# ZooMEISTER/vickers-hardness-Unet

Measured on AMD Instinct MI355X. Metric: 512x512 images/sec (train fwd+bwd), higher is better.
Workload: dtype bf16

## Files before the change

### vickers-hardness-unet_amd/csrc/conv_halo.hip

```cpp
#include <stdlib.h>
#include <string.h>

#include <string>
#include <type_traits>

#include "vk_common.h"

#ifdef VK_STAMP
#define VK_T(var) { __builtin_amdgcn_sched_barrier(0); const unsigned long long t_ = __builtin_amdgcn_s_memtime(); __builtin_amdgcn_s_waitcnt(0xC07F); __builtin_amdgcn_sched_barrier(0); var = t_; }
#else
#define VK_T(var)
#endif

namespace vk {

struct HaloSrc {
  const void* ptr;
  const float* scale;
  const float* shift;
  int C, up, relu;
  uint32_t bytes;
};

#ifndef VK_EPI_BATCH_READS
#define VK_EPI_BATCH_READS 1
#endif
#ifndef VK_COLP_DEFER_STATS
#define VK_COLP_DEFER_STATS 1
#endif
#ifndef VK_COLQ_ILV
#define VK_COLQ_ILV 1
#endif
#ifndef VK_COLQ_DIAG
#define VK_COLQ_DIAG 0
#endif
#ifndef VK_COLQ_PRE
#define VK_COLQ_PRE 1
#endif
struct HaloParams {
  HaloSrc s0, s1;
  const void* w;
  uint32_t w_bytes;
  void* y0;
  void* y1;
  int ld0, ld1, split;
  double* stats;
  int N, H, W, K, C, flip, accumulate, pool2;
  int Hi, Wi;
  int tiles_x, tiles_y, nchunks;
  unsigned long long* stamps;
  int kyn;
  int ksplit;
  size_t slab_bytes;
  float* slab;
  int dbg;
  const void* bnr_z;
  const float* bnr_scale;
  const float* bnr_shift;
  double* bnr_sums;
  const void* bnr_mask;
};

template <typename T, int TH, int BN, int WGM, int WGN>
struct HaloCfg {
  using Tr = ElemTraits<T>;
  static constexpr int EB = Tr::kBytes;
  static constexpr int VE = Tr::kVec;
  static constexpr int CK = 64 / EB;
  static constexpr int HW_ = 18, HH = TH + 2, HPIX = HH * HW_;
  static constexpr int APS = 96;
  static constexpr int A_BYTES = HPIX * APS;
  static constexpr int B_BYTES = 3 * BN * 64;
  static constexpr int NPV = (HPIX * 4 + 255) / 256;
  static constexpr int NBV = (3 * BN * 4 + 255) / 256;
  static constexpr int BM = TH * 16;
  static constexpr int WR = TH / WGM;
  static constexpr int WCH = BN / WGN;
  static constexpr int TP = WR, TC = WCH / 16;
  static constexpr int ESB = BN * EB + 16;
  static constexpr int EVPR = BN / VE;
  static constexpr int ERPP = 256 / EVPR;
  static constexpr int EPASS = BM / ERPP;
  static constexpr int RED_OFF = BM * ESB;
  static constexpr int MAIN = A_BYTES + 2 * B_BYTES;
  static constexpr int ESLOTS = (BN / VE > 16) ? 4 * 4 / (BN / VE / 16) : 4 * 4;
  static constexpr int EPI = RED_OFF + ESLOTS * BN * 2 * 4;
  static constexpr int SMEM = MAIN > EPI ? MAIN : EPI;
  static_assert(WGM * WGN == 4 && TH % WGM == 0 && BN % (16 * WGN) == 0, "wave layout");
  static_assert(EPASS >= 1, "epilogue mapping");
  static_assert(SMEM <= 160 * 1024, "main-loop / epilogue LDS image exceeds the 160 KiB of a CU");
};

__device__ __forceinline__ int swz(int row) { return ((row >> 2) & 1) << 1; }

__device__ __forceinline__ int halo_group(int tid) {
  const int g = tid >> 2;
  return (g & ~3) | ((g & 1) << 1) | ((g >> 1) & 1);
}


template <typename T, int TH, int BN, int TP, int TC, int NT = 256, bool PRE = false, int OS = 1>
__device__ __forceinline__ void halo_epilogue(char* smem, f32x4_t (&acc)[TC][TP], const HaloParams& p, int n, int y0, int x0, int n0,
                                              int wrow0, int wch0, int py = 0, int px = 0, double* defer = nullptr) {
  using Tr = ElemTraits<T>;
  constexpr int EB = Tr::kBytes, VE = Tr::kVec;
  constexpr int BM = TH * 16;
  constexpr int ESB = BN * EB + 16;
  constexpr int EVPR = BN / VE, ERPP = NT / EVPR, EPASS = BM / ERPP, NW = NT / 64;
  constexpr int RED_OFF = BM * ESB;
  static_assert(BM % ERPP == 0 && EVPR <= 64, "epilogue mapping");
  const int tid = threadIdx.x, lane = tid & 63, wave = tid >> 6;
  const int li = lane & 15, kg = lane >> 4;

  const int e_row = tid / EVPR;
  const int e_vec = (EVPR == 16 && EB == 2) ? (((tid & 15) + ((e_row & 1) ? 15 : 0)) & 15) : tid % EVPR;
  const int col0 = n0 + e_vec * VE;
  const bool col_ok = col0 < p.K;
  char* yb = (char*)p.y0;
  int ld = p.ld0, colx = col0;
  bool first_part = true;
  if (p.split > 0 && col0 >= p.split) { yb = (char*)p.y1; ld = p.ld1; colx = col0 - p.split; first_part = false; }
  float s1[VE], s2[VE];
#pragma unroll
  for (int j = 0; j < VE; ++j) { s1[j] = 0.f; s2[j] = 0.f; }
  const bool bnr = p.bnr_z != nullptr && first_part && col_ok;
  const bool ext_mask = p.bnr_mask != nullptr;
  float bsc[VE], bsh[VE];
  if (bnr && !ext_mask) {
#pragma unroll
    for (int j = 0; j < VE; ++j) { bsc[j] = p.bnr_scale[colx + j]; bsh[j] = p.bnr_shift[colx + j]; }
  }
  auto finish = [&](float (&f)[VE], size_t elem_off, const u32x4_t* pre_old, const u32x4_t* pre_z, const u32x4_t* pre_m = nullptr) {
    u32x4_t* gp = reinterpret_cast<u32x4_t*>(yb + elem_off * EB);
    if (p.accumulate) {
      float o[VE];
      Vec16<T>::unpack(pre_old ? *pre_old : *gp, o);
#pragma unroll
      for (int j = 0; j < VE; ++j) f[j] += o[j];
    }
    u32x4_t v = Vec16<T>::pack(f);
    Vec16<T>::unpack(v, f);
    if (bnr) {
      float zf[VE];
// ... 73 lines not shown
        for (int q = 0; q < 4; ++q) {
          const int row = (2 * py + (q >> 1)) * 16 + 2 * px + (q & 1);
          float t[VE];
          Vec16<T>::unpack(*reinterpret_cast<const u32x4_t*>(smem + row * ESB + e_vec * 16), t);
#pragma unroll
          for (int j = 0; j < VE; ++j) f[j] += t[j];
        }
        finish(f, (((size_t)n * Hh + y) * Wh + x) * ld + colx, nullptr, nullptr);
      }
    }
  } else if (p.accumulate || p.bnr_z != nullptr) {
#pragma unroll
    for (int ps = 0; ps < EPASS; ++ps) {
      const int row = e_row + ps * ERPP;
      const int y = OS * (y0 + (row >> 4)) + py, x = OS * (x0 + (row & 15)) + px;
      if (y < p.H && x < p.W && col_ok) {
        const u32x4_t raw = *reinterpret_cast<const u32x4_t*>(smem + row * ESB + e_vec * 16);
        const size_t eoff = (((size_t)n * p.H + y) * p.W + x) * ld + colx;
        float f[VE];
        Vec16<T>::unpack(raw, f);
        if (PRE) finish(f, eoff, &oldv[ps], &zv[ps], PRE_M ? &mv[ps] : nullptr);
        else finish(f, eoff, nullptr, nullptr);
      }
    }
  } else {
    constexpr int RB = VK_EPI_BATCH_READS ? (EPASS < 8 ? EPASS : 8) : 1;
    u32x4_t raws[RB];
#pragma unroll
    for (int ps = 0; ps < EPASS; ++ps) {
      if (ps % RB == 0) {
#pragma unroll
        for (int q = 0; q < RB; ++q)
          if (ps + q < EPASS) raws[q] = *reinterpret_cast<const u32x4_t*>(smem + (e_row + (ps + q) * ERPP) * ESB + e_vec * 16);
      }
      const int row = e_row + ps * ERPP;
      const int y = OS * (y0 + (row >> 4)) + py, x = OS * (x0 + (row & 15)) + px;
      if (y < p.H && x < p.W && col_ok) {
        const u32x4_t raw = raws[ps % RB];
        const size_t eoff = (((size_t)n * p.H + y) * p.W + x) * ld + colx;
        if (p.stats) {
          float f[VE];
          Vec16<T>::unpack(raw, f);
#pragma unroll
          for (int j = 0; j < VE; ++j) { s1[j] += f[j]; s2[j] += f[j] * f[j]; }
        }
        *reinterpret_cast<u32x4_t*>(yb + eoff * EB) = raw;
      }
    }
  }
  if (p.stats || p.bnr_sums) {
    if (p.bnr_sums && !bnr) {
#pragma unroll
      for (int j = 0; j < VE; ++j) { s1[j] = 0.f; s2[j] = 0.f; }
    }
#pragma unroll
    for (int j = 0; j < VE; ++j) {
      if (EVPR <= 1) { s1[j] += dpp_f<0xB1>(s1[j]); s2[j] += dpp_f<0xB1>(s2[j]); }
      if (EVPR <= 2) { s1[j] += dpp_f<0x4E>(s1[j]); s2[j] += dpp_f<0x4E>(s2[j]); }
      if (EVPR <= 4) { s1[j] += dpp_f<0x124>(s1[j]); s2[j] += dpp_f<0x124>(s2[j]); }
      if (EVPR <= 8) { s1[j] += dpp_f<0x128>(s1[j]); s2[j] += dpp_f<0x128>(s2[j]); }
    }
    float* red = reinterpret_cast<float*>(smem + RED_OFF);
    constexpr int RPS = EVPR > 16 ? EVPR / 16 : 1, NSLOT = NW * 4 / RPS;
    static_assert(EVPR <= 32, "partial-sum slots");
    if (EVPR > 16 || li < EVPR) {
      const int slot = (wave * 4 + kg) / RPS;
#pragma unroll
      for (int j = 0; j < VE; ++j) {
        red[(slot * BN + e_vec * VE + j) * 2 + 0] = s1[j];
        red[(slot * BN + e_vec * VE + j) * 2 + 1] = s2[j];
      }
    }
    __syncthreads();
    if (tid < BN && n0 + tid < p.K) {
      float a = 0.f, b = 0.f;
#pragma unroll
      for (int w = 0; w < NSLOT; ++w) { a += red[(w * BN + tid) * 2]; b += red[(w * BN + tid) * 2 + 1]; }
      if (defer) {
        defer[0] += (double)a;
        defer[1] += (double)b;
      } else if (p.bnr_sums) {
        const int kc = p.ld0;
        if (n0 + tid < kc) {
          double* sp = p.bnr_sums + (size_t)(blockIdx.x % VK_STATS_REPLICAS) * 2 * kc;
          atomicAdd(sp + n0 + tid, (double)a);
          atomicAdd(sp + kc + n0 + tid, (double)b);
        }
      } else {
        double* sp = p.stats + (size_t)(blockIdx.x % VK_STATS_REPLICAS) * 2 * p.K;
        atomicAdd(sp + n0 + tid, (double)a);
        atomicAdd(sp + p.K + n0 + tid, (double)b);
      }
    }
  }
}

template <int BN>
__device__ __forceinline__ void stats_flush(const HaloParams& p, int n0, double (&d)[2]) {
  const int tid = threadIdx.x;
  if (tid < BN && n0 + tid < p.K) {
    if (p.bnr_sums) {
      const int kc = p.ld0;
      if (n0 + tid < kc) {
        double* sp = p.bnr_sums + (size_t)(blockIdx.x % VK_STATS_REPLICAS) * 2 * kc;
        atomicAdd(sp + n0 + tid, d[0]);
        atomicAdd(sp + kc + n0 + tid, d[1]);
      }
    } else if (p.stats) {
      double* sp = p.stats + (size_t)(blockIdx.x % VK_STATS_REPLICAS) * 2 * p.K;
      atomicAdd(sp + n0 + tid, d[0]);
      atomicAdd(sp + p.K + n0 + tid, d[1]);
    }
  }
  d[0] = 0.0;
  d[1] = 0.0;
}

template <typename T, int TH, int BN, int WGM, int WGN>
__global__ __launch_bounds__(256, 2) void conv3x3_halo_kernel(const HaloParams p) {
  using Cfg = HaloCfg<T, TH, BN, WGM, WGN>;
  constexpr int EB = Cfg::EB, VE = Cfg::VE, CK = Cfg::CK, HPIX = Cfg::HPIX, NPV = Cfg::NPV, NBV = Cfg::NBV;
  constexpr int TP = Cfg::TP, TC = Cfg::TC, APS = Cfg::APS;

  extern __shared__ __attribute__((aligned(16))) char smem[];
  char* const Abuf = smem;
  char* const Bbuf = smem + Cfg::A_BYTES;
  const int tid = threadIdx.x, lane = tid & 63, wave = tid >> 6;

  int bt = blockIdx.x;
  if ((gridDim.x & 7) == 0) bt = (bt & 7) * (int)(gridDim.x >> 3) + (bt >> 3);
  const int tx = bt % p.tiles_x;
  bt /= p.tiles_x;
  const int ty = bt % p.tiles_y;
  const int n = bt / p.tiles_y;
  const int y0 = ty * TH, x0 = tx * 16;
  const int n0 = blockIdx.y * BN;

  const __amdgpu_buffer_rsrc_t rs0 = make_rsrc(p.s0.ptr, p.s0.bytes);
  const __amdgpu_buffer_rsrc_t rs1 = make_rsrc(p.s1.ptr ? p.s1.ptr : p.s0.ptr, p.s1.ptr ? p.s1.bytes : 0u);
  const __amdgpu_buffer_rsrc_t rsw = make_rsrc(p.w, p.w_bytes);

  const int hv = tid & 3;
  const int hgrp = halo_group(tid);
  int h_full[NPV], h_half[NPV];
  const int Hh = p.H >> 1, Wh = p.W >> 1;
#pragma unroll
  for (int i = 0; i < NPV; ++i) {
    const int hp = hgrp + i * 64;
    const int hy = hp / 18, hx = hp - hy * 18;
    const int y = y0 - 1 + hy, x = x0 - 1 + hx;
    const bool ok = hp < HPIX && (unsigned)y < (unsigned)p.H && (unsigned)x < (unsigned)p.W;
    h_full[i] = ok ? (n * p.H + y) * p.W + x : -1;
    h_half[i] = ok ? (n * Hh + (y >> 1)) * Wh + (x >> 1) : -1;
  }
  int b_toff[NBV];
  int b_s[NBV];
#pragma unroll
  for (int i = 0; i < NBV; ++i) {
    const int idx = tid + i * 256;
    b_s[i] = idx / (BN * 4);
    b_toff[i] = idx < 3 * BN * 4 ? (idx - b_s[i] * (BN * 4)) * 16 : -1;
  }
  const uint32_t slab_bytes = (uint32_t)p.K * 64u;

  u32x4_t areg[NPV], breg0[NBV], breg1[NBV];
  float sc[VE], sh[VE];
  bool aff = false, relu = false;

  auto load_halo = [&](int cc) {
    const int c = cc * CK;
    const bool first = c < p.s0.C;
    const HaloSrc& sd = first ? p.s0 : p.s1;
    const int cl = (first ? c : c - p.s0.C) + hv * VE;
    aff = sd.scale != nullptr;
    relu = sd.relu != 0;
    if (aff) {
#pragma unroll
      for (int j = 0; j < VE; j += 4) {
        const f32x4_t s4 = *reinterpret_cast<const f32x4_t*>(sd.scale + cl + j);
        const f32x4_t h4 = *reinterpret_cast<const f32x4_t*>(sd.shift + cl + j);
#pragma unroll
        for (int e = 0; e < 4; ++e) { sc[j + e] = s4[e]; sh[j + e] = h4[e]; }
      }
    }
    const bool up = sd.up != 0;
#pragma unroll
    for (int i = 0; i < NPV; ++i) {
      const int pix = up ? h_half[i] : h_full[i];
      const uint32_t off = (uint32_t)(pix * sd.C + cl) * (uint32_t)EB;
      if (first) areg[i] = buf_load16(rs0, pix >= 0 ? off : kOOB);
      else areg[i] = buf_load16(rs1, pix >= 0 ? off : kOOB);
    }
// ... 1265 lines not shown

template <typename T>
__global__ __launch_bounds__(256, 3) void stem7x7_kernel(const HaloParams p) {
  using Cfg = ColCfg<T, 16, 64, 4, 1, false>;
  static_assert(sizeof(T) == 2, "16-bit types: a pixel of the NHWC4 input is 8 bytes");
  constexpr int NV = (StemTile::ROWS * StemTile::VPR + 255) / 256;
  extern __shared__ __attribute__((aligned(16))) char smem[];
  const int tid = threadIdx.x, lane = tid & 63;
  const int wave = __builtin_amdgcn_readfirstlane(tid >> 6);
  int bt = blockIdx.x;
  if ((gridDim.x & 7) == 0) bt = (bt & 7) * (int)(gridDim.x >> 3) + (bt >> 3);
  const int tx = bt % p.tiles_x;
  bt /= p.tiles_x;
  const int ty = bt % p.tiles_y;
  const int n = bt / p.tiles_y;
  const int y0 = ty * 16, x0 = tx * 16;
  const __amdgpu_buffer_rsrc_t rs0 = make_rsrc(p.s0.ptr, p.s0.bytes);
  const __amdgpu_buffer_rsrc_t rsw = make_rsrc(p.w, p.w_bytes);

  u32x4_t areg[NV];
#pragma unroll
  for (int i = 0; i < NV; ++i) {
    const int v = tid + i * 256;
    const int ry = v / StemTile::VPR, vc = v - ry * StemTile::VPR;
    const int y = 2 * y0 - 3 + ry, x = 2 * x0 - 4 + 2 * vc;
    const bool ok = v < StemTile::ROWS * StemTile::VPR && (unsigned)y < (unsigned)p.Hi && (unsigned)x < (unsigned)p.Wi;
    areg[i] = buf_load16(rs0, ok ? (uint32_t)((n * p.Hi + y) * p.Wi + x) * 8u : kOOB);
  }
  const int li = lane & 15, kg = lane >> 4;
  typedef __attribute__((address_space(3))) void lds_void;
  char* const Wl = smem + StemTile::W_OFF;
#pragma unroll
  for (int i = 0; i < 7; ++i) {
    const int pc = wave * 7 + i, r = pc >> 2, a = pc & 3;
    const uint32_t voff = (uint32_t)((((a * 16 + li) * 7 + r) * 32 + kg * 8) * 2);
    __builtin_amdgcn_raw_ptr_buffer_load_lds(rsw, (lds_void*)(Wl + pc * 1024), 16, voff, 0, 0, 0);
  }
#pragma unroll
  for (int i = 0; i < NV; ++i) {
    const int v = tid + i * 256;
    if (v >= StemTile::ROWS * StemTile::VPR) continue;
    const int ry = v / StemTile::VPR, vc = v - ry * StemTile::VPR;
    char* row = smem + ry * StemTile::PITCH;
    if (vc > 0) *reinterpret_cast<u32x2_t*>(row + (2 * vc - 1) * 8) = u32x2_t{areg[i][0], areg[i][1]};
    *reinterpret_cast<u32x2_t*>(row + (2 * vc) * 8) = u32x2_t{areg[i][2], areg[i][3]};
  }
  __syncthreads();

  const int wrow0 = wave * 4;
  f32x4_t acc[4][4];
#pragma unroll
  for (int a = 0; a < 4; ++a)
#pragma unroll
    for (int b = 0; b < 4; ++b) acc[a][b] = f32x4_t{0.f, 0.f, 0.f, 0.f};
  const char* const xl = smem + (2 * wrow0) * StemTile::PITCH + 16 * (li + kg);
  const char* const wl = Wl + lane * 16;
#pragma unroll
  for (int r = 0; r < 7; ++r) {
    u32x4_t X[4], Wc[4];
#pragma unroll
    for (int a = 0; a < 4; ++a) Wc[a] = *reinterpret_cast<const u32x4_t*>(wl + (4 * r + a) * 1024);
#pragma unroll
    for (int b = 0; b < 4; ++b) X[b] = *reinterpret_cast<const u32x4_t*>(xl + (2 * b + r) * StemTile::PITCH);
#pragma unroll
    for (int a = 0; a < 4; ++a)
#pragma unroll
      for (int b = 0; b < 4; ++b) acc[a][b] = Mma<T>::run(Wc[a], X[b], acc[a][b]);
  }
  __syncthreads();
  halo_epilogue<T, 16, 64, 4, 4, 256, false>(smem, acc, p, n, y0, x0, 0, wrow0, 0);
}

int stem_tile_launch(vk_dtype dt, int N, int H, int W, const void* x4, const void* wp, void* y, double* stats, hipStream_t st) {
  if (dt == VK_F32 || getenv("VK_NO_STEM_TILE")) return VK_ERR_UNSUPPORTED;
  if ((size_t)N * H * W * 8 >= (1ull << 31)) return VK_ERR_UNSUPPORTED;
  HaloParams p;
  memset((void*)&p, 0, sizeof(p));
  p.s0 = HaloSrc{x4, nullptr, nullptr, 4, 0, 0, (uint32_t)((size_t)N * H * W * 8)};
  p.w = wp;
  p.w_bytes = 64u * 7u * 32u * 2u;
  p.y0 = y;
  p.ld0 = 64;
  p.stats = stats;
  p.N = N; p.H = H / 2; p.W = W / 2; p.K = 64; p.C = 4;
  p.Hi = H; p.Wi = W;
  p.tiles_x = (p.W + 15) / 16;
  p.tiles_y = (p.H + 15) / 16;
  using Cfg = ColCfg<bf16_t, 16, 64, 4, 1, false>;
  constexpr int MAIN = StemTile::W_OFF + StemTile::W_BYTES;
  constexpr int SMEM = MAIN > Cfg::EPI ? MAIN : Cfg::EPI;
  const dim3 grid((unsigned)(N * p.tiles_y * p.tiles_x));
  vkh::ProfScope ps("stem_tile_16b", st, 2.0 * (double)N * p.H * p.W * 64.0 * 147.0, ((double)N * H * W * 4.0 + (double)N * p.H * p.W * 64.0) * 2.0);
  if (dt == VK_BF16) hipLaunchKernelGGL(stem7x7_kernel<bf16_t>, grid, dim3(256), SMEM, st, p);
  else hipLaunchKernelGGL(stem7x7_kernel<f16_t>, grid, dim3(256), SMEM, st, p);
  VK_CHECK_HIP(hipGetLastError());
  return VK_OK;
}

template <typename T, int BN>
struct C16Cfg {
  static constexpr int TH = 16, HPIX = 18 * 18;
  static constexpr int APS = 48;
  static constexpr int A_BYTES = HPIX * APS + 64;
  static constexpr int BS = 336;
  static constexpr int B_BYTES = BN * BS;
  static constexpr int TP = 4, TC = BN / 16;
  static constexpr int ESB = BN * 2 + 16;
  static constexpr int EPI = 256 * ESB + 4 * 4 * BN * 2 * 4;
  static constexpr int MAIN = A_BYTES + B_BYTES;
  static constexpr int SMEM = MAIN > EPI ? MAIN : EPI;
};

template <typename T, int BN>
__global__ __launch_bounds__(256) void conv3x3_c16_kernel(const HaloParams p) {
  using Cfg = C16Cfg<T, BN>;
  constexpr int TH = 16, HPIX = Cfg::HPIX, APS = Cfg::APS, BS = Cfg::BS, TP = Cfg::TP, TC = Cfg::TC, VE = 8;
  static_assert(sizeof(T) == 2, "C16 kernel is for 16-bit element types (fp32 uses the generic kernel with 16-channel chunks)");
  extern __shared__ __attribute__((aligned(16))) char smem[];
  char* const Abuf = smem;
  char* const Bbuf = smem + Cfg::A_BYTES;
  const int tid = threadIdx.x, lane = tid & 63, wave = tid >> 6;
  int bt = blockIdx.x;
  if ((gridDim.x & 7) == 0) bt = (bt & 7) * (int)(gridDim.x >> 3) + (bt >> 3);
  const int tx = bt % p.tiles_x;
  bt /= p.tiles_x;
  const int ty = bt % p.tiles_y;
  const int n = bt / p.tiles_y;
  const int y0 = ty * TH, x0 = tx * 16;
  const int n0 = blockIdx.y * BN;
  const __amdgpu_buffer_rsrc_t rs0 = make_rsrc(p.s0.ptr, p.s0.bytes);
  const __amdgpu_buffer_rsrc_t rsw = make_rsrc(p.w, p.w_bytes);

  const bool aff = p.s0.scale != nullptr, relu = p.s0.relu != 0;
  const int hv = (tid >> 3) & 1;
  const int hgrp = (tid & 7) | ((tid >> 4) << 3);
  float sc[VE], sh[VE];
#pragma unroll
  for (int j = 0; j < VE; ++j) {
    sc[j] = aff ? p.s0.scale[hv * VE + j] : 1.f;
    sh[j] = aff ? p.s0.shift[hv * VE + j] : 0.f;
  }
  constexpr int NPV = (HPIX * 2 + 255) / 256;
  u32x4_t areg[NPV];
  bool aok[NPV];
#pragma unroll
  for (int i = 0; i < NPV; ++i) {
    const int hp = hgrp + i * 128;
    const int hy = hp / 18, hx = hp - hy * 18;
    const int y = y0 - 1 + hy, x = x0 - 1 + hx;
    aok[i] = hp < HPIX && (unsigned)y < (unsigned)p.H && (unsigned)x < (unsigned)p.W;
    const uint32_t off = (uint32_t)(((n * p.H + y) * p.W + x) * 16 + hv * VE) * 2u;
    areg[i] = buf_load16(rs0, aok[i] ? off : kOOB);
  }
  constexpr int NBV = (BN * 18 + 255) / 256;
  u32x4_t breg[NBV];
#pragma unroll
  for (int i = 0; i < NBV; ++i) {
    const int idx = tid + i * 256;
    const int row = idx / 18, v = idx - row * 18;
    const int tap = p.flip ? 8 - (v >> 1) : (v >> 1);
    const bool ok = idx < BN * 18 && n0 + row < p.K;
    breg[i] = buf_load16(rsw, ok ? (uint32_t)(((n0 + row) * 9 + tap) * 16 + (v & 1) * VE) * 2u : kOOB);
  }
  if (tid < 4) *reinterpret_cast<u32x4_t*>(Abuf + HPIX * APS + tid * 16) = u32x4_t{0, 0, 0, 0};
  if (tid < BN) {
    *reinterpret_cast<u32x4_t*>(Bbuf + tid * BS + 288) = u32x4_t{0, 0, 0, 0};
// ... 262 lines not shown
  issue(jb + 1, pre[1]);
  issue(jb + 2, pre[2]);
  if (BNR) z_issue(POOL ? ys + 1 : ys, zq[0]);
  write_row(jb - 1, pre[3]);
  issue(jb + 3, pre[3]);
  write_row(jb, pre[0]);
  auto row = [&](int y, auto ph_c) {
    constexpr int PH = decltype(ph_c)::value;
    if constexpr (!UP) {
      constexpr int S = (PH + 1) & 3;
      write_row(y + 1, pre[S]);
      issue(y + 4, pre[PH & 3]);
    } else if constexpr ((PH & 1) == 1) {
      constexpr int M1 = ((PH + 1) >> 1) & 3;
      const int m1 = (y + 1) >> 1;
      write_row(m1, pre[M1]);
      issue(m1 + 3, pre[(M1 + 3) & 3]);
    }
    constexpr int ZC = POOL ? ((PH >> 1) & 1) : (PH & 1);
    if constexpr (BNR && (!POOL || (PH & 1) == 1)) z_issue(POOL ? y + 2 : y + 1, zq[ZC ^ 1]);
    f32x4_t acc[TC];
#pragma unroll
    for (int a = 0; a < TC; ++a) acc[a] = f32x4_t{0.f, 0.f, 0.f, 0.f};
#pragma unroll
    for (int st = 0; st < NSTEP; ++st) {
      int addr;
      if (CIN == 16) {
        const int vrow = y - 1 + fr_r16[st];
        addr = fr_r16[st] < 0 ? Cfg::ZERO_OFF : (vrow & 3) * ROWB + fr_off16[st];
      } else {
        const int r = st / 3, sxx = st - r * 3;
        const int vrow = y - 1 + r;
        const int jr = UP ? (vrow >> 1) : vrow;
        const int pix = UP ? ((li + sxx + 1) >> 1) : (li + sxx);
        addr = (jr & 3) * ROWB + pix * APS + fr_base32;
      }
      const u32x4_t xf = *reinterpret_cast<const u32x4_t*>(ring + addr);
#pragma unroll
      for (int a = 0; a < TC; ++a) acc[a] = Mma<T>::run(wf[st][a], xf, acc[a]);
    }
#if !(VK_STREAM_DIAG & 16)
    __builtin_amdgcn_sched_barrier(0);
#endif
    const bool y_ok = y < p.H;
#pragma unroll
    for (int a = 0; a < TC; ++a) {
      const int ch = a * 16 + kg * 4;
      float f[4] = {acc[a][0], acc[a][1], acc[a][2], acc[a][3]};
      u32x2_t pk = round_t(f);
      if constexpr (POOL) {
        if constexpr ((PH & 1) == 0) {
#pragma unroll
          for (int e = 0; e < 4; ++e) prev[a][e] = f[e];
        } else {
          float t[4];
#pragma unroll
          for (int e = 0; e < 4; ++e) {
            const float pn = dpp_f<0xB1>(prev[a][e]), cn = dpp_f<0xB1>(f[e]);
            t[e] = ((prev[a][e] + pn) + f[e]) + cn;
          }
          const u32x2_t pk2 = round_t(t);
          finish(a, t, pk2, y_ok ? out_off(a, y) : kOOB, lane_stores && y_ok, zq[ZC][a]);
        }
      } else {
        finish(a, f, pk, y_ok ? out_off(a, y) : kOOB, lane_stores && y_ok, zq[ZC][a]);
      }
    }
  };
  constexpr int UF = UP ? 8 : 4;
  for (int yb = ys; yb < ye; yb += UF) {
    row(yb, std::integral_constant<int, 0>{});
    row(yb + 1, std::integral_constant<int, 1>{});
    row(yb + 2, std::integral_constant<int, 2>{});
    row(yb + 3, std::integral_constant<int, 3>{});
    if constexpr (UP) {
      row(yb + 4, std::integral_constant<int, 4>{});
      row(yb + 5, std::integral_constant<int, 5>{});
      row(yb + 6, std::integral_constant<int, 6>{});
      row(yb + 7, std::integral_constant<int, 7>{});
    }
  }

  if (want_sums) {
    double* const sp = (p.bnr_sums ? p.bnr_sums : p.stats) + (size_t)(strip % VK_STATS_REPLICAS) * 2 * ld;
#pragma unroll
    for (int a = 0; a < TC; ++a)
#pragma unroll
      for (int e = 0; e < 4; ++e) {
        const float u = row16_sum(s1[a][e]), v = row16_sum(s2[a][e]);
        const int ch = a * 16 + kg * 4 + e;
        if (li == 0 && ch < ld) {
          atomicAdd(sp + ch, (double)u);
          atomicAdd(sp + ld + ch, (double)v);
        }
      }
  }
}

struct TailCfg {
  static constexpr int S_STRIDE = 96, A1_STRIDE = 48, A2_PS = 20;
  static constexpr int S_BYTES = 144 * S_STRIDE;
  static constexpr int A1_BYTES = 400 * A1_STRIDE + 64;
  static constexpr int A2_BYTES = 324 * A2_PS * 4;
  static constexpr int SMEM = S_BYTES + A1_BYTES + A2_BYTES;
};

struct TailParams {
  const void* src;
  const float* s0;
  const float* h0;
  const void* w1;
  const float* s1;
  const float* h1;
  const void* w2;
  const float* s2;
  const float* h2;
  const float* hw;
  const float* hb;
  float* logits;
  int N, H, W;
  uint32_t src_bytes;
};

template <typename T>
__global__ __launch_bounds__(256) void dec4_tail_eval_kernel(const TailParams p) {
  using Cfg = TailCfg;
  static_assert(sizeof(T) == 2, "16-bit element types");
  constexpr int VE = 8;
  extern __shared__ __attribute__((aligned(16))) char smem[];
  char* const Sb = smem;
  char* const A1 = smem + Cfg::S_BYTES;
  float* const A2 = reinterpret_cast<float*>(smem + Cfg::S_BYTES + Cfg::A1_BYTES);
  const int tid = threadIdx.x, lane = tid & 63, wave = tid >> 6, li = lane & 15, kg = lane >> 4;
  const int tiles_x = p.W >> 4, tiles_y = p.H >> 4;
  int bt = blockIdx.x;
  const int tx0 = bt % tiles_x;
  bt /= tiles_x;
  const int ty0 = bt % tiles_y;
  const int n = bt / tiles_y;
  const int y0 = ty0 * 16, x0 = tx0 * 16;
  const int Hs = p.H >> 1, Ws = p.W >> 1;
  const int sy0 = (y0 >> 1) - 2, sx0 = (x0 >> 1) - 2;
  const __amdgpu_buffer_rsrc_t rss = make_rsrc(p.src, p.src_bytes);

  u32x4_t wf1[9], wf2[5];
#pragma unroll
  for (int st = 0; st < 9; ++st) {
    const int pos = kg ^ (((li >> 2) & 1) << 1);
    wf1[st] = *reinterpret_cast<const u32x4_t*>((const char*)p.w1 + ((st * 16 + li) * 4 + pos) * 16);
  }
#pragma unroll
  for (int st = 0; st < 5; ++st) {
    const int tap = 2 * st + (kg >> 1);
    wf2[st] = u32x4_t{0, 0, 0, 0};
    if (tap < 9) wf2[st] = *reinterpret_cast<const u32x4_t*>((const char*)p.w2 + ((li * 9 + tap) * 16 + (kg & 1) * VE) * 2);
  }
  float sc1[8], sh1[8], sc2[4], sh2[4];
#pragma unroll
  for (int e = 0; e < 4; ++e) {
    sc1[e] = p.s1[kg * 4 + e]; sh1[e] = p.h1[kg * 4 + e];
    sc1[4 + e] = 0.f; sh1[4 + e] = 0.f;
    sc2[e] = p.s2[kg * 4 + e]; sh2[e] = p.h2[kg * 4 + e];
  }
  if (tid < 4) *reinterpret_cast<u32x4_t*>(A1 + 400 * Cfg::A1_STRIDE + tid * 16) = u32x4_t{0, 0, 0, 0};

  {
    float sc0[VE], sh0[VE];
// ... 402 lines not shown
  static const std::string tag_f = std::string("stream_16b_c") + std::to_string(CIN) + (UP ? "up" : "") + "_k" + std::to_string(TC * 16);
  static const std::string tag_d = tag_f + "_dgrad";
  const std::string& tag = p.flip ? tag_d : tag_f;
  const double in_px = (double)p.N * (p.H >> (UP ? 1 : 0)) * (p.W >> (UP ? 1 : 0));
  const double out_px = (double)p.N * p.H * p.W * (p.pool2 ? 0.25 : 1.0);
  const double bytes = (in_px * CIN + out_px * p.K * (p.bnr_z ? 2.0 : 1.0) + 9.0 * p.K * CIN) * 2.0;
  vkh::ProfScope ps(tag.c_str(), st, 2.0 * (double)p.N * p.H * p.W * p.K * 9.0 * CIN, bytes);
  hipLaunchKernelGGL((conv3x3_stream_kernel<T, CIN, TC, UP, MODE>), grid, dim3(256), Cfg::SMEM, st, q);
  VK_CHECK_HIP(hipGetLastError());
  return VK_OK;
}

template <typename T>
static int stream_try(const HaloParams& p, hipStream_t st) {
  if (getenv("VK_NO_STREAM")) return VK_ERR_UNSUPPORTED;
  if (p.s1.ptr || p.accumulate || p.split || p.ld0 != p.K) return VK_ERR_UNSUPPORTED;
  const bool up = p.s0.up != 0, bnr = p.bnr_z != nullptr, pool = p.pool2 != 0;
  if ((pool || up) && ((p.H | p.W) & 1)) return VK_ERR_UNSUPPORTED;
  const bool fwd = !p.flip && !bnr && !pool;
  if (fwd && p.C == 32 && up && p.K == 16) return launch_stream<T, 32, 1, true, 0>(p, st);
  if (fwd && p.C == 16 && !up && p.K == 16) return launch_stream<T, 16, 1, false, 0>(p, st);
  if (fwd && p.C == 32 && !up && p.K == 32) return launch_stream<T, 32, 2, false, 0>(p, st);
  if (p.flip && !p.s0.scale && bnr && !pool && p.C == 16 && p.K == 16) return launch_stream<T, 16, 1, false, 2>(p, st);
  if (p.flip && !p.s0.scale && bnr && !pool && p.C == 32 && p.K == 32) return launch_stream<T, 32, 2, false, 2>(p, st);
  if (p.flip && !p.s0.scale && bnr && pool && p.C == 16 && p.K == 32) return launch_stream<T, 16, 2, false, 3>(p, st);
  return VK_ERR_UNSUPPORTED;
}

int conv3x3_halo_try(const vk_conv_desc* d, const void* w, int packed, void* y, void* y1, int split_k1, int accumulate, double* stats,
                     int pool2, const vk_bnr* bnr, hipStream_t st, void* workspace, size_t workspace_bytes) {
  const bool s2 = d->stride == 2 && !d->transposed && d->H == 2 * d->Ho && d->W == 2 * d->Wo && d->K >= 128 && !d->src0.up && !d->src1.ptr &&
                  !pool2 && !bnr && !accumulate && !split_k1 && !getenv("VK_NO_S2_TILE");
  const bool s2d = d->stride == 2 && d->transposed && d->Ho == 2 * d->H && d->Wo == 2 * d->W && d->K >= 64 && d->K % 64 == 0 && !d->src0.up &&
                   !d->src1.ptr && !d->src0.scale && !pool2 && !bnr && !split_k1 && !getenv("VK_NO_S2_TILE");
  if (d->R != 3 || d->S != 3 || d->pad != 1) return VK_ERR_UNSUPPORTED;
  if (!s2 && !s2d && (d->stride != 1 || d->H != d->Ho || d->W != d->Wo)) return VK_ERR_UNSUPPORTED;
  const int eb = d->dtype == VK_F32 ? 4 : 2;
  const int ck = 64 / eb;
  const int C = d->src0.C + (d->src1.ptr ? d->src1.C : 0);
  const bool c16 = (eb == 2) && C == 16 && !d->src1.ptr && !d->src0.up && !s2 && !s2d;
  if (c16 ? packed : !packed) return VK_ERR_UNSUPPORTED;
  if (!c16 && (d->src0.C % ck || (d->src1.ptr && d->src1.C % ck))) return VK_ERR_UNSUPPORTED;
  if (d->K % 16) return VK_ERR_UNSUPPORTED;
  if (pool2 && ((d->H | d->W) & 1)) return VK_ERR_UNSUPPORTED;
  if (d->src1.ptr && d->src1.up) return VK_ERR_UNSUPPORTED;
  if ((size_t)d->N * d->H * d->W * C * eb >= (1ull << 31) || (size_t)d->N * d->H * d->W >= (1ull << 31)) return VK_ERR_UNSUPPORTED;
  if (s2d && (size_t)d->N * d->Ho * d->Wo * d->K * eb >= (1ull << 32)) return VK_ERR_UNSUPPORTED;
  HaloParams p;
  auto mk = [&](const vk_src& s) {
    HaloSrc h;
    h.ptr = s.ptr; h.scale = s.scale; h.shift = s.shift; h.C = s.C; h.up = s.up; h.relu = s.relu;
    h.bytes = s.ptr ? (uint32_t)((size_t)d->N * (d->H >> s.up) * (d->W >> s.up) * s.C * eb) : 0u;
    return h;
  };
  p.s0 = mk(d->src0);
  if (d->src1.ptr) p.s1 = mk(d->src1);
  else p.s1 = HaloSrc{nullptr, nullptr, nullptr, 0, 0, 0, 0u};
  p.w = w;
  p.w_bytes = (uint32_t)((size_t)d->K * 9 * C * eb);
  p.y0 = y; p.y1 = y1; p.split = split_k1;
  p.ld0 = split_k1 ? split_k1 : d->K;
  p.ld1 = split_k1 ? d->K - split_k1 : 0;
  p.stats = stats;
  p.N = d->N; p.H = d->Ho; p.W = d->Wo; p.K = d->K; p.C = C;
  p.Hi = d->H; p.Wi = d->W;
  p.flip = d->transposed;
  p.accumulate = accumulate;
  p.pool2 = pool2;
  p.ksplit = 1;
  p.kyn = 0;
  p.slab = (reinterpret_cast<uintptr_t>(workspace) & 15) ? nullptr : (float*)workspace;
  p.slab_bytes = p.slab ? workspace_bytes : 0;
  p.stamps = nullptr;
  p.dbg = getenv("VK_COL_DBG") ? atoi(getenv("VK_COL_DBG")) : 0;
  if (p.dbg & 1) p.w_bytes = 0;
#ifdef VK_STAMP
  { extern unsigned long long* g_vk_stamp_buf; p.stamps = g_vk_stamp_buf; }
#endif
  p.bnr_z = bnr ? bnr->z : nullptr;
  p.bnr_scale = bnr ? bnr->scale : nullptr;
  p.bnr_shift = bnr ? bnr->shift : nullptr;
  p.bnr_sums = bnr ? bnr->sums : nullptr;
  p.bnr_mask = bnr ? bnr->mask : nullptr;
  p.nchunks = c16 ? 1 : C / ck;
  if (p.bnr_mask && (c16 || s2 || s2d || pool2)) return VK_ERR_UNSUPPORTED;
  if (eb == 2 && !s2 && !s2d && !p.bnr_mask && (c16 || C == 32)) {
    const int rc = d->dtype == VK_BF16 ? stream_try<bf16_t>(p, st) : stream_try<f16_t>(p, st);
    if (rc != VK_ERR_UNSUPPORTED) return rc;
  }
  if (c16) {
    if (d->dtype == VK_BF16) return d->K >= 32 ? launch_c16<bf16_t, 32>(p, st) : launch_c16<bf16_t, 16>(p, st);
    return d->K >= 32 ? launch_c16<f16_t, 32>(p, st) : launch_c16<f16_t, 16>(p, st);
  }
  p.tiles_x = p.tiles_y = 0;
  if (s2d) {
    p.flip = 0;
    const long tiles = (long)d->N * ((d->H + 7) / 8) * ((d->W + 15) / 16);
    const bool wide = d->K % 128 == 0 && tiles * (d->K / 128) >= 256;
    switch (d->dtype) {
      case VK_F32: return wide ? launch_s2dg<float, 128>(p, st) : launch_s2dg<float, 64>(p, st);
      case VK_BF16: return wide ? launch_s2dg<bf16_t, 128>(p, st) : launch_s2dg<bf16_t, 64>(p, st);
      case VK_F16: return wide ? launch_s2dg<f16_t, 128>(p, st) : launch_s2dg<f16_t, 64>(p, st);
    }
    return VK_ERR_ARG;
  }
  if (s2) {
    p.slab = nullptr;
    p.slab_bytes = 0;
    switch (d->dtype) {
      case VK_F32: return launch_col<float, 8, 128, 2, 4, false, 1, 0, 2>(p, st);
      case VK_BF16: return launch_col<bf16_t, 8, 128, 2, 4, false, 1, 0, 2>(p, st);
      case VK_F16: return launch_col<f16_t, 8, 128, 2, 4, false, 1, 0, 2>(p, st);
    }
    return VK_ERR_ARG;
  }
  switch (d->dtype) {
    case VK_F32: return halo_select<float>(p, st);
    case VK_BF16: return halo_select<bf16_t>(p, st);
    case VK_F16: return halo_select<f16_t>(p, st);
  }
  return VK_ERR_ARG;
}

}

extern "C" int vk_dec4_tail_eval(vk_dtype dtype, int N, int H, int W, const vk_src* src, const void* w1_pack, const float* scale1,
                                 const float* shift1, const void* w2_plain, const float* scale2, const float* shift2, const float* head_w9x16,
                                 const float* head_bias, float* logits, void* stream) {
  return vk::dec4_tail_eval_impl(dtype, N, H, W, src, w1_pack, scale1, shift1, w2_plain, scale2, shift2, head_w9x16, head_bias, logits,
                                 (hipStream_t)stream);
}
```

### vickers-hardness-unet_amd/csrc/elementwise.hip

```cpp
#include <math.h>

#include "vk_common.h"

namespace vk {

static inline int grid_for(size_t work_items, int block = 256, int max_blocks = 256 * 16) {
  size_t b = (work_items + block - 1) / block;
  if (b > (size_t)max_blocks) b = max_blocks;
  if (b < 1) b = 1;
  return (int)b;
}

template <typename T>
__global__ void k_input_transform(int N, int H, int W, const float* __restrict__ x, T* __restrict__ x4) {
  const size_t HW = (size_t)H * W;
  const float* xn = x + (size_t)blockIdx.y * 3 * HW;
  T* on = x4 + (size_t)blockIdx.y * HW * 4;
  for (size_t hw = blockIdx.x * (size_t)blockDim.x + threadIdx.x; hw < HW; hw += (size_t)gridDim.x * blockDim.x) {
    const float r = xn[hw], g = xn[HW + hw], b = xn[2 * HW + hw];
    if constexpr (sizeof(T) == 4) {
      *reinterpret_cast<f32x4_t*>(on + hw * 4) = f32x4_t{r, g, b, 0.f};
    } else {
      float f[8] = {r, g, b, 0.f, 0.f, 0.f, 0.f, 0.f};
      const u32x4_t pk = Vec16<T>::pack(f);
      *reinterpret_cast<u32x2_t*>(on + hw * 4) = u32x2_t{pk[0], pk[1]};
    }
  }
}

__global__ __launch_bounds__(256) void k_bn_finalize(int C, int train, const double* __restrict__ stats, double count,
                                                     const float* __restrict__ gamma, const float* __restrict__ beta, float* running_mean,
                                                     float* running_var, float eps, float momentum, float* scale, float* shift,
                                                     float* save_mean, float* save_invstd) {
  static_assert(VK_STATS_REPLICAS == 32, "lane mapping assumes 32 replicas");
  const int c = blockIdx.x * 8 + (threadIdx.x >> 5);
  const int r = threadIdx.x & 31;
  double s1 = 0.0, s2 = 0.0;
  if (train && c < C) {
    s1 = stats[(size_t)r * 2 * C + c];
    s2 = stats[(size_t)r * 2 * C + C + c];
  }
  const bool fin = r == 0 && c < C;
  const float ga = fin ? gamma[c] : 0.f, be = fin ? beta[c] : 0.f;
  const float rm0 = fin && running_mean ? running_mean[c] : 0.f, rv0 = fin && running_var ? running_var[c] : 0.f;
#pragma unroll
  for (int o = 16; o > 0; o >>= 1) {
    s1 += __shfl_xor(s1, o, 64);
    s2 += __shfl_xor(s2, o, 64);
  }
  if (!fin) return;
  double mean, var;
  if (train) {
    mean = s1 / count;
    var = s2 / count - mean * mean;
    if (var < 0.0) var = 0.0;
    if (running_mean) {
      const double unb = count > 1.0 ? var * count / (count - 1.0) : var;
      running_mean[c] = (float)((1.0 - momentum) * rm0 + momentum * mean);
      running_var[c] = (float)((1.0 - momentum) * rv0 + momentum * unb);
    }
  } else {
    mean = rm0;
    var = rv0;
  }
  const float invstd = (float)(1.0 / sqrt(var + (double)eps));
  const float sc = ga * invstd;
  scale[c] = sc;
  shift[c] = be - (float)mean * sc;
  if (save_mean) save_mean[c] = (float)mean;
  if (save_invstd) save_invstd[c] = invstd;
}

template <typename T>
__global__ void k_bn_relu_maxpool(int N, int H, int W, int C, const T* __restrict__ z, const float* __restrict__ scale,
                                  const float* __restrict__ shift, T* __restrict__ pooled, uint8_t* __restrict__ argmax) {
  constexpr int VE = ElemTraits<T>::kVec;
  const int Hp = H / 2, Wp = W / 2, CV = C / VE;
  const unsigned t = blockIdx.x * blockDim.x + threadIdx.x;
  if (t < (unsigned)(Wp * CV)) {
    const int pw = (int)(t / (unsigned)CV), cv = (int)(t - (unsigned)pw * CV);
    const int ph = blockIdx.y, n = blockIdx.z;
    const size_t i = (((size_t)n * Hp + ph) * Wp + pw) * CV + cv;
    float sc[VE], sh[VE], best[VE];
    int bi[VE];
#pragma unroll
    for (int j = 0; j < VE; ++j) {
      sc[j] = scale[cv * VE + j];
      sh[j] = shift[cv * VE + j];
      best[j] = -INFINITY;
      bi[j] = 0;
    }
#pragma unroll
    for (int r = 0; r < 3; ++r) {
      const int h = 2 * ph - 1 + r;
// ... 146 lines not shown
  float sc[VE], sh[VE], s1[VE], s2[VE];
#pragma unroll
  for (int j = 0; j < VE; ++j) {
    sc[j] = scale[cv * VE + j];
    sh[j] = shift[cv * VE + j];
    s1[j] = 0.f;
    s2[j] = 0.f;
  }
  const int pw0 = (w & 1) ? (w - 1) / 2 : w / 2, npw = (w & 1) ? 2 : 1;
  if (active) {
    for (int hr = 0; hr < PB_ROWS; ++hr) {
      const int h = blockIdx.y * PB_ROWS + hr;
      if (h >= H) break;
      const size_t i = (((size_t)n * H + h) * W + w) * CV + cv;
      float g[VE], zf[VE];
      Vec16<T>::unpack(*reinterpret_cast<const u32x4_t*>(dy + i * VE), g);
      Vec16<T>::unpack(*reinterpret_cast<const u32x4_t*>(z + i * VE), zf);
      const int ph0 = (h & 1) ? (h - 1) / 2 : h / 2, nph = (h & 1) ? 2 : 1;
      float acc[VE];
#pragma unroll
      for (int j = 0; j < VE; ++j) acc[j] = 0.f;
      for (int a = 0; a < nph; ++a) {
        const int ph = ph0 + a;
        if (ph >= Hp) continue;
        const int r = h - (2 * ph - 1);
        for (int b = 0; b < npw; ++b) {
          const int pw = pw0 + b;
          if (pw >= Wp) continue;
          const int code = r * 3 + (w - (2 * pw - 1));
          const size_t pi = (((size_t)n * Hp + ph) * Wp + pw) * C + cv * VE;
          uint32_t am[VE];
          if (VE == 8) {
            const u32x2_t q = *reinterpret_cast<const u32x2_t*>(argmax + pi);
#pragma unroll
            for (int j = 0; j < VE; ++j) am[j] = (q[j >> 2] >> (8 * (j & 3))) & 0xffu;
          } else {
            const uint32_t q = *reinterpret_cast<const uint32_t*>(argmax + pi);
#pragma unroll
            for (int j = 0; j < VE; ++j) am[j] = (q >> (8 * j)) & 0xffu;
          }
          float pg[VE];
          Vec16<T>::unpack(*reinterpret_cast<const u32x4_t*>(dpool + pi), pg);
#pragma unroll
          for (int j = 0; j < VE; ++j)
            if (am[j] == (uint32_t)code) acc[j] += pg[j];
        }
      }
#pragma unroll
      for (int j = 0; j < VE; ++j) g[j] += acc[j];
      u32x4_t v = Vec16<T>::pack(g);
      Vec16<T>::unpack(v, g);
#pragma unroll
      for (int j = 0; j < VE; ++j) {
        if (!(fmaf(zf[j], sc[j], sh[j]) > 0.f)) g[j] = 0.f;
        s1[j] += g[j];
        s2[j] += g[j] * zf[j];
      }
      *reinterpret_cast<u32x4_t*>(dy + i * VE) = Vec16<T>::pack(g);
    }
  }
  __shared__ float red[256 * 2 * 8];
#pragma unroll
  for (int j = 0; j < VE; ++j) {
    red[(tid * VE + j) * 2] = active ? s1[j] : 0.f;
    red[(tid * VE + j) * 2 + 1] = active ? s2[j] : 0.f;
  }
  __syncthreads();
  const int rows = 256 / CV;
  for (int c = tid; c < C; c += 256) {
    const int ccv = c / VE, cj = c % VE;
    double a = 0.0, b = 0.0;
    for (int r = 0; r < rows; ++r) {
      const int tt = r * CV + ccv;
      a += red[(tt * VE + cj) * 2];
      b += red[(tt * VE + cj) * 2 + 1];
    }
    double* sp = sums + (size_t)((blockIdx.x + blockIdx.y * gridDim.x) % VK_STATS_REPLICAS) * 2 * C;
    atomicAdd(sp + c, a);
    atomicAdd(sp + C + c, b);
  }
}

template <typename T, int MASK>
__device__ __forceinline__ void masked_grad(const T* dy, const T* z, const T* mask_src, size_t off, const float* sc,
                                            const float* sh, float* g, float* zf) {
  constexpr int VE = ElemTraits<T>::kVec;
  Vec16<T>::unpack(*reinterpret_cast<const u32x4_t*>(dy + off), g);
  Vec16<T>::unpack(*reinterpret_cast<const u32x4_t*>(z + off), zf);
  if (MASK == 1) {
#pragma unroll
    for (int j = 0; j < VE; ++j)
      if (!(fmaf(zf[j], sc[j], sh[j]) > 0.f)) g[j] = 0.f;
  } else if (MASK == 2) {
    float m[VE];
    Vec16<T>::unpack(*reinterpret_cast<const u32x4_t*>(mask_src + off), m);
#pragma unroll
    for (int j = 0; j < VE; ++j)
      if (!(m[j] > 0.f)) g[j] = 0.f;
  }
}

template <typename T, int MASK>
__global__ __launch_bounds__(256) void k_bn_bwd_reduce(size_t pixels, int C, const T* __restrict__ dy, const T* __restrict__ z,
                                                       const float* __restrict__ scale, const float* __restrict__ shift,
                                                       const T* __restrict__ mask_src, double* sums) {
  constexpr int VE = ElemTraits<T>::kVec;
  const int CV = C / VE;
  const int rows = 256 / CV;
  const int tid = threadIdx.x;
  const int cv = tid % CV, row = tid / CV;
  const bool active = row < rows;
  float sc[VE], sh[VE], s1[VE], s2[VE];
#pragma unroll
  for (int j = 0; j < VE; ++j) {
    sc[j] = (MASK == 1) ? scale[cv * VE + j] : 1.f;
    sh[j] = (MASK == 1) ? shift[cv * VE + j] : 0.f;
    s1[j] = 0.f;
    s2[j] = 0.f;
  }
  if (active) {
    const size_t stride = (size_t)gridDim.x * rows;
    size_t p = (size_t)blockIdx.x * rows + row;
    for (; p + 3 * stride < pixels; p += 4 * stride) {
      float g[4][VE], zf[4][VE];
#pragma unroll
      for (int u = 0; u < 4; ++u) masked_grad<T, MASK>(dy, z, mask_src, (p + u * stride) * C + cv * VE, sc, sh, g[u], zf[u]);
#pragma unroll
      for (int u = 0; u < 4; ++u)
#pragma unroll
        for (int j = 0; j < VE; ++j) { s1[j] += g[u][j]; s2[j] += g[u][j] * zf[u][j]; }
    }
    for (; p < pixels; p += stride) {
      float g[VE], zf[VE];
      masked_grad<T, MASK>(dy, z, mask_src, p * C + cv * VE, sc, sh, g, zf);
#pragma unroll
      for (int j = 0; j < VE; ++j) { s1[j] += g[j]; s2[j] += g[j] * zf[j]; }
    }
  }
  __shared__ float red[256 * 2 * 8];
#pragma unroll
  for (int j = 0; j < VE; ++j) {
    red[(tid * VE + j) * 2] = active ? s1[j] : 0.f;
    red[(tid * VE + j) * 2 + 1] = active ? s2[j] : 0.f;
  }
  __syncthreads();
  for (int c = tid; c < C; c += 256) {
    const int ccv = c / VE, cj = c % VE;
    double a = 0.0, b = 0.0;
    for (int r = 0; r < rows; ++r) {
      const int t = r * CV + ccv;
      a += red[(t * VE + cj) * 2];
      b += red[(t * VE + cj) * 2 + 1];
    }
    double* sp = sums + (size_t)(blockIdx.x % VK_STATS_REPLICAS) * 2 * C;
    atomicAdd(sp + c, a);
    atomicAdd(sp + C + c, b);
  }
}

__global__ __launch_bounds__(256) void k_bn_bwd_coeffs(int C, const double* __restrict__ sums, double count, const float* __restrict__ gamma,
                                                       const float* __restrict__ save_mean, const float* __restrict__ save_invstd, float* dgamma,
                                                       float* dbeta, float* coef) {
  const int c = blockIdx.x * 8 + (threadIdx.x >> 5);
  const int q = threadIdx.x & 31;
  double sg = 0.0, sgz = 0.0;
  if (c < C) {
    sg = sums[(size_t)q * 2 * C + c];
    sgz = sums[(size_t)q * 2 * C + C + c];
  }
  const bool fin = q == 0 && c < C;
  const double mu = fin ? save_mean[c] : 0.f, r = fin ? save_invstd[c] : 0.f, ga = fin ? gamma[c] : 0.f;
  const float dg0 = fin ? dgamma[c] : 0.f, db0 = fin ? dbeta[c] : 0.f;
#pragma unroll
  for (int o = 16; o > 0; o >>= 1) {
    sg += __shfl_xor(sg, o, 64);
    sgz += __shfl_xor(sgz, o, 64);
  }
  if (!fin) return;
  const double dg = r * (sgz - mu * sg);
  const double db = sg;
  dgamma[c] = dg0 + (float)dg;
  dbeta[c] = db0 + (float)db;
  const double a = ga * r;
  const double b = -ga * r * r * dg / count;
  const double cc = -a * db / count - b * mu;
  coef[c] = (float)a;
  coef[C + c] = (float)b;
  coef[2 * C + c] = (float)cc;
}

__global__ __launch_bounds__(256) void k_bn_bwd_coeffs_frozen(int C, const double* __restrict__ sums, const float* __restrict__ gamma,
                                                              const float* __restrict__ save_mean, const float* __restrict__ save_invstd,
                                                              float* dgamma, float* dbeta, float* coef) {
  const int c = blockIdx.x * 8 + (threadIdx.x >> 5);
  const int q = threadIdx.x & 31;
  double sg = 0.0, sgz = 0.0;
  if (c < C) {
    sg = sums[(size_t)q * 2 * C + c];
    sgz = sums[(size_t)q * 2 * C + C + c];
  }
#pragma unroll
  for (int o = 16; o > 0; o >>= 1) {
    sg += __shfl_xor(sg, o, 64);
    sgz += __shfl_xor(sgz, o, 64);
  }
  if (q != 0 || c >= C) return;
  const float r = save_invstd[c];
  dgamma[c] += (float)((double)r * (sgz - (double)save_mean[c] * sg));
  dbeta[c] += (float)sg;
  coef[c] = gamma[c] * r;
  coef[C + c] = 0.f;
  coef[2 * C + c] = 0.f;
}

template <typename T, int MASK>
__global__ __launch_bounds__(256) void k_bn_bwd_apply(size_t pixels, int C, const T* __restrict__ dy, const T* __restrict__ z,
                                                      const float* __restrict__ scale, const float* __restrict__ shift, const T* __restrict__ mask_src,
                                                      const float* __restrict__ coef, const double* __restrict__ sums, double count,
                                                      const float* __restrict__ gamma, const float* __restrict__ save_mean,
                                                      const float* __restrict__ save_invstd, float* dgamma, float* dbeta, T* __restrict__ dz, T* g_out,
                                                      int g_acc) {
  constexpr int VE = ElemTraits<T>::kVec;
  constexpr int U = 2;
  const int CV = C / VE;
  const size_t total = pixels * CV;
  const size_t stride = (size_t)gridDim.x * blockDim.x;
  const size_t t0 = blockIdx.x * (size_t)blockDim.x + threadIdx.x;
  const int c0 = (int)(t0 % CV) * VE;
  __shared__ float cf[3][512];
  if (coef) {
    for (int c = threadIdx.x; c < C; c += blockDim.x) {
      cf[0][c] = coef[c];
      cf[1][c] = coef[C + c];
      cf[2][c] = coef[2 * C + c];
    }
  } else {
    static_assert(VK_STATS_REPLICAS == 32, "replica mapping");
    for (int c8 = threadIdx.x; c8 < C * 8; c8 += blockDim.x) {
      const int c = c8 >> 3, q0 = (c8 & 7) * 4;
      double sg = 0.0, sgz = 0.0;
#pragma unroll
      for (int q = 0; q < 4; ++q) {
        sg += sums[(size_t)(q0 + q) * 2 * C + c];
        sgz += sums[(size_t)(q0 + q) * 2 * C + C + c];
      }
#pragma unroll
      for (int o = 4; o > 0; o >>= 1) {
        sg += __shfl_xor(sg, o, 64);
        sgz += __shfl_xor(sgz, o, 64);
      }
      if ((c8 & 7) == 0) {
        const float mu = save_mean[c], r = save_invstd[c], ga = gamma[c];
        const float d = (float)(sgz - (double)mu * sg);
        const float sgf = (float)sg, inv = (float)(1.0 / count);
        const float dg = r * d;
        const float a = ga * r, b = -a * r * dg * inv;
        cf[0][c] = a;
        cf[1][c] = b;
        cf[2][c] = -a * sgf * inv - b * mu;
        if (blockIdx.x == 0) {
          dgamma[c] += dg;
          dbeta[c] += sgf;
        }
      }
    }
  }
  __syncthreads();
  float sc[VE], sh[VE], ca[VE], cb[VE], cc[VE];
#pragma unroll
  for (int j = 0; j < VE; ++j) {
    sc[j] = (MASK == 1) ? scale[c0 + j] : 1.f;
    sh[j] = (MASK == 1) ? shift[c0 + j] : 0.f;
    ca[j] = cf[0][c0 + j];
    cb[j] = cf[1][c0 + j];
    cc[j] = cf[2][c0 + j];
  }
  for (size_t i = t0; i < total; i += U * stride) {
    float g[U][VE], zf[U][VE];
#pragma unroll
    for (int u = 0; u < U; ++u)
      if (i + u * stride < total) masked_grad<T, MASK>(dy, z, mask_src, (i + u * stride) * VE, sc, sh, g[u], zf[u]);
#pragma unroll
    for (int u = 0; u < U; ++u) {
      const size_t k = i + u * stride;
      if (k >= total) continue;
      float o[VE];
#pragma unroll
      for (int j = 0; j < VE; ++j) o[j] = fmaf(ca[j], g[u][j], fmaf(cb[j], zf[u][j], cc[j]));
      *reinterpret_cast<u32x4_t*>(dz + k * VE) = Vec16<T>::pack(o);
      if (g_out) {
        u32x4_t* gp = reinterpret_cast<u32x4_t*>(g_out + k * VE);
        if (g_acc) {
          float old[VE];
          Vec16<T>::unpack(*gp, old);
#pragma unroll
          for (int j = 0; j < VE; ++j) g[u][j] += old[j];
        }
        *gp = Vec16<T>::pack(g[u]);
      }
    }
  }
}

template <typename T>
__global__ void k_upsample2x_bwd(int N, int H, int W, int C, const T* __restrict__ d_up, T* __restrict__ d_low, int acc) {
  constexpr int VE = ElemTraits<T>::kVec;
  const int Hl = H / 2, Wl = W / 2, CV = C / VE;
  const size_t total = (size_t)N * Hl * Wl * CV;
  for (size_t i = blockIdx.x * (size_t)blockDim.x + threadIdx.x; i < total; i += (size_t)gridDim.x * blockDim.x) {
    const int cv = (int)(i % CV);
    size_t t = i / CV;
    const int wl = (int)(t % Wl);
    t /= Wl;
    const int hl = (int)(t % Hl);
    const int n = (int)(t / Hl);
    float s[VE];
#pragma unroll
    for (int j = 0; j < VE; ++j) s[j] = 0.f;
#pragma unroll
    for (int a = 0; a < 2; ++a)
#pragma unroll
      for (int b = 0; b < 2; ++b) {
        float f[VE];
        Vec16<T>::unpack(*reinterpret_cast<const u32x4_t*>(d_up + (((size_t)n * H + 2 * hl + a) * W + 2 * wl + b) * C + cv * VE), f);
#pragma unroll
        for (int j = 0; j < VE; ++j) s[j] += f[j];
      }
    u32x4_t* op = reinterpret_cast<u32x4_t*>(d_low + i * VE);
    if (acc) {
      float o[VE];
      Vec16<T>::unpack(*op, o);
#pragma unroll
      for (int j = 0; j < VE; ++j) s[j] += o[j];
    }
    *op = Vec16<T>::pack(s);
  }
}

template <typename T>
__device__ __forceinline__ void load_act16(const T* p, const float* sc, const float* sh, bool affine, bool relu, float* a) {
  constexpr int VE = ElemTraits<T>::kVec;
#pragma unroll
  for (int v = 0; v < 16 / VE; ++v) Vec16<T>::unpack(*reinterpret_cast<const u32x4_t*>(p + v * VE), a + v * VE);
  if (affine) {
#pragma unroll
    for (int j = 0; j < 16; ++j) {
      a[j] = fmaf(a[j], sc[j], sh[j]);
      if (relu) a[j] = fmaxf(a[j], 0.f);
    }
  }
}

template <typename T>
__global__ __launch_bounds__(256) void k_head_fwd(int N, int H, int W, int tiles_x, int tiles_y, const T* __restrict__ z,
                                                  const float* __restrict__ scale, const float* __restrict__ shift, int relu,
                                                  const float* __restrict__ w, const float* __restrict__ bias, float* __restrict__ logits) {
  constexpr int VE = ElemTraits<T>::kVec, VPP = 16 / VE;
  constexpr int PS = 20;
  __shared__ __attribute__((aligned(16))) float tile[18 * 18 * PS];
  const int tid = threadIdx.x;
  int bt = blockIdx.x;
  const int tx0 = bt % tiles_x;
  bt /= tiles_x;
  const int ty0 = bt % tiles_y;
  const int n = bt / tiles_y;
  const int y0 = ty0 * 16, x0 = tx0 * 16;
  const bool affine = scale != nullptr;
  const int vec = tid % VPP;
  float sc[VE], sh[VE];
#pragma unroll
  for (int j = 0; j < VE; ++j) { sc[j] = affine ? scale[vec * VE + j] : 1.f; sh[j] = affine ? shift[vec * VE + j] : 0.f; }
  constexpr int NHV = (324 * VPP + 255) / 256;
  u32x4_t raw[NHV];
  bool inb[NHV];
#pragma unroll
  for (int i = 0; i < NHV; ++i) {
    const int v = tid + i * 256;
    const int hp = v / VPP;
    const int hy = hp / 18, hx = hp - hy * 18;
    const int y = y0 - 1 + hy, x = x0 - 1 + hx;
    inb[i] = v < 324 * VPP && (unsigned)y < (unsigned)H && (unsigned)x < (unsigned)W;
    raw[i] = u32x4_t{0, 0, 0, 0};
// ... 619 lines not shown
  VK_CHECK_ARG(x && x4 && N > 0 && H > 0 && W > 0, "vk_input_transform: bad argument");
  hipStream_t st = (hipStream_t)stream;
  vkh::ProfScope ps_("input_transform", st, 0.0, (double)N * H * W * (12.0 + 4.0 * (dtype == VK_F32 ? 4.0 : 2.0)));
  VK_CHECK_ARG(N <= 65535, "vk_input_transform: N too large for the launch grid");
  DISPATCH_T(dtype, hipLaunchKernelGGL(k_input_transform<T>, dim3(grid_for((size_t)H * W, 256, 1024), (unsigned)N), dim3(256), 0, st, N, H, W, x, (T*)x4));
  VK_CHECK_HIP(hipGetLastError());
  return VK_OK;
}

extern "C" int vk_bn_finalize(int C, int train, const double* stats, double count, const float* gamma, const float* beta,
                              float* running_mean, float* running_var, float eps, float momentum, float* scale, float* shift,
                              float* save_mean, float* save_invstd, void* stream) {
  VK_CHECK_ARG(C > 0 && gamma && beta && scale && shift, "vk_bn_finalize: null argument");
  VK_CHECK_ARG(train ? (stats != nullptr && count > 0) : (running_mean && running_var), "vk_bn_finalize: missing statistics");
  vkh::ProfScope ps_("bn_finalize", (hipStream_t)stream, 0.0, (double)C * 40.0);
  hipLaunchKernelGGL(k_bn_finalize, dim3((C + 7) / 8), dim3(256), 0, (hipStream_t)stream, C, train, stats, count, gamma, beta,
                     running_mean, running_var, eps, momentum, scale, shift, save_mean, save_invstd);
  VK_CHECK_HIP(hipGetLastError());
  return VK_OK;
}

extern "C" int vk_bn_relu_maxpool(vk_dtype dtype, int N, int H, int W, int C, const void* z, const float* scale,
                                  const float* shift, void* pooled, uint8_t* argmax, void* stream) {
  VK_CHECK_ARG(z && scale && shift && pooled && argmax, "vk_bn_relu_maxpool: null argument");
  VK_CHECK_ARG(H % 2 == 0 && W % 2 == 0 && C % 8 == 0, "vk_bn_relu_maxpool: H, W even and C %% 8 == 0 required");
  hipStream_t st = (hipStream_t)stream;
  vkh::ProfScope ps_("bn_relu_maxpool", st, 0.0, (double)N * H * W * C * (dtype == VK_F32 ? 4.0 : 2.0) * 1.25 + (double)N * H * W * C / 4.0);
  VK_CHECK_ARG(N <= 65535 && H / 2 <= 65535, "vk_bn_relu_maxpool: N or H too large for the launch grid");
  DISPATCH_T(dtype, hipLaunchKernelGGL(k_bn_relu_maxpool<T>, dim3((unsigned)(((W / 2) * (C / ElemTraits<T>::kVec) + 255) / 256), (unsigned)(H / 2), (unsigned)N),
                                       dim3(256), 0, st, N, H, W, C, (const T*)z, scale, shift, (T*)pooled, argmax));
  VK_CHECK_HIP(hipGetLastError());
  return VK_OK;
}

extern "C" int vk_maxpool_bwd(vk_dtype dtype, int N, int H, int W, int C, const void* dpool, const uint8_t* argmax, void* dy,
                              void* stream) {
  VK_CHECK_ARG(dpool && argmax && dy && C % 8 == 0, "vk_maxpool_bwd: bad argument");
  hipStream_t st = (hipStream_t)stream;
  vkh::ProfScope ps_("maxpool_bwd", st, 0.0, (double)N * H * W * C * (dtype == VK_F32 ? 4.0 : 2.0) * 2.25 + (double)N * H * W * C / 4.0);
  VK_CHECK_ARG(N <= 65535 && H <= 65535 && H % 2 == 0 && W % 2 == 0, "vk_maxpool_bwd: N or H too large for the launch grid, or odd size");
  DISPATCH_T(dtype, hipLaunchKernelGGL(k_maxpool_bwd<T>, dim3((unsigned)((W * (C / ElemTraits<T>::kVec) + 255) / 256), (unsigned)H, (unsigned)N), dim3(256), 0, st,
                                       N, H, W, C, (const T*)dpool, argmax, (T*)dy));
  VK_CHECK_HIP(hipGetLastError());
  return VK_OK;
}

extern "C" int vk_maxpool_bwd_bn_reduce(vk_dtype dtype, int N, int H, int W, int C, const void* dpool, const uint8_t* argmax, const void* z,
                                        const float* scale, const float* shift, void* dy, double* sums, void* stream) {
  VK_CHECK_ARG(dpool && argmax && z && scale && shift && dy && sums, "vk_maxpool_bwd_bn_reduce: null argument");
  VK_CHECK_ARG(H % 2 == 0 && W % 2 == 0 && C % 8 == 0, "vk_maxpool_bwd_bn_reduce: H, W even and C %% 8 == 0 required");
  const int cv = C / (dtype == VK_F32 ? 4 : 8);
  VK_CHECK_ARG(cv <= 256 && 256 % cv == 0, "vk_maxpool_bwd_bn_reduce: C=%d unsupported", C);
  VK_CHECK_ARG(N <= 65535 && H <= 65535 * vk::PB_ROWS, "vk_maxpool_bwd_bn_reduce: N or H too large for the launch grid");
  hipStream_t st = (hipStream_t)stream;
  const double eb = dtype == VK_F32 ? 4.0 : 2.0;
  vkh::ProfScope ps_("maxpool_bwd_bn_reduce", st, 0.0, (double)N * H * W * C * eb * 3.25 + (double)N * H * W * C / 4.0);
  DISPATCH_T(dtype, hipLaunchKernelGGL(k_maxpool_bwd_bn_reduce<T>, dim3((unsigned)((W * cv + 255) / 256), (unsigned)((H + PB_ROWS - 1) / PB_ROWS), (unsigned)N),
                                       dim3(256), 0, st, N, H, W, C, (const T*)dpool, argmax, (const T*)z, scale, shift, (T*)dy, sums));
  VK_CHECK_HIP(hipGetLastError());
  return VK_OK;
}

extern "C" int vk_bn_add_relu(vk_dtype dtype, size_t pixels, int C, const void* z, const float* scale, const float* shift,
                              const void* res, const float* rscale, const float* rshift, void* out, void* stream) {
  VK_CHECK_ARG(z && scale && shift && res && out && C % 8 == 0, "vk_bn_add_relu: bad argument");
  hipStream_t st = (hipStream_t)stream;
  vkh::ProfScope ps_("bn_add_relu", st, 0.0, (double)pixels * C * (dtype == VK_F32 ? 4.0 : 2.0) * 3.0);
  VK_CHECK_ARG(C <= 512, "vk_bn_add_relu: C=%d unsupported", C);
  DISPATCH_T(dtype, hipLaunchKernelGGL(k_bn_add_relu<T>, dim3(grid_for((pixels * (C / ElemTraits<T>::kVec) + 3) / 4)), dim3(256), 0, st, pixels, C,
                                       (const T*)z, scale, shift, (const T*)res, rscale, rshift, (T*)out));
  VK_CHECK_HIP(hipGetLastError());
  return VK_OK;
}

template <typename T>
static int launch_bn_bwd_reduce(size_t pixels, int C, const void* dy, const void* z, int mask_mode, const float* scale,
                                const float* shift, const void* mask_src, double* sums, hipStream_t st) {
  const int CV = C / ElemTraits<T>::kVec;
  const int rows = 256 / CV;
  size_t nb = (pixels + (size_t)rows * 16 - 1) / ((size_t)rows * 16);
  if (nb > 2048) nb = 2048;
  if (nb < 1) nb = 1;
  dim3 grid((unsigned)nb), block(256);
  if (mask_mode == 0) hipLaunchKernelGGL((k_bn_bwd_reduce<T, 0>), grid, block, 0, st, pixels, C, (const T*)dy, (const T*)z, scale, shift, (const T*)mask_src, sums);
  else if (mask_mode == 1) hipLaunchKernelGGL((k_bn_bwd_reduce<T, 1>), grid, block, 0, st, pixels, C, (const T*)dy, (const T*)z, scale, shift, (const T*)mask_src, sums);
  else hipLaunchKernelGGL((k_bn_bwd_reduce<T, 2>), grid, block, 0, st, pixels, C, (const T*)dy, (const T*)z, scale, shift, (const T*)mask_src, sums);
  return VK_OK;
}

extern "C" int vk_bn_bwd_reduce(vk_dtype dtype, size_t pixels, int C, const void* dy, const void* z, int mask_mode,
                                const float* scale, const float* shift, const void* mask_src, double* sums, void* stream) {
  VK_CHECK_ARG(dy && z && sums, "vk_bn_bwd_reduce: null argument");
  VK_CHECK_ARG(mask_mode >= 0 && mask_mode <= 2, "vk_bn_bwd_reduce: mask_mode %d", mask_mode);
  VK_CHECK_ARG(mask_mode != 1 || (scale && shift), "vk_bn_bwd_reduce: mask_mode 1 needs scale/shift");
  VK_CHECK_ARG(mask_mode != 2 || mask_src, "vk_bn_bwd_reduce: mask_mode 2 needs mask_src");
  VK_CHECK_ARG(C % 8 == 0 && C <= 512, "vk_bn_bwd_reduce: C=%d unsupported", C);
  hipStream_t st = (hipStream_t)stream;
  vkh::ProfScope ps_("bn_bwd_reduce", st, 0.0, (double)pixels * C * (dtype == VK_F32 ? 4.0 : 2.0) * (mask_mode == 2 ? 3.0 : 2.0));
  DISPATCH_T(dtype, launch_bn_bwd_reduce<T>(pixels, C, dy, z, mask_mode, scale, shift, mask_src, sums, st));
  VK_CHECK_HIP(hipGetLastError());
  return VK_OK;
}

extern "C" int vk_bn_bwd_coeffs(int C, const double* sums, double count, const float* gamma, const float* save_mean,
                                const float* save_invstd, float* dgamma, float* dbeta, float* coef_abc, void* stream) {
  VK_CHECK_ARG(sums && gamma && save_mean && save_invstd && dgamma && dbeta && coef_abc, "vk_bn_bwd_coeffs: null argument");
  vkh::ProfScope ps_("bn_bwd_coeffs", (hipStream_t)stream, 0.0, (double)C * 48.0);
  hipLaunchKernelGGL(k_bn_bwd_coeffs, dim3((C + 7) / 8), dim3(256), 0, (hipStream_t)stream, C, sums, count, gamma, save_mean,
                     save_invstd, dgamma, dbeta, coef_abc);
  VK_CHECK_HIP(hipGetLastError());
  return VK_OK;
}

extern "C" int vk_bn_bwd_coeffs_frozen(int C, const double* sums, const float* gamma, const float* running_mean, const float* running_invstd,
                                       float* dgamma, float* dbeta, float* coef_abc, void* stream) {
  VK_CHECK_ARG(sums && gamma && running_mean && running_invstd && dgamma && dbeta && coef_abc, "vk_bn_bwd_coeffs_frozen: null argument");
  vkh::ProfScope ps_("bn_bwd_coeffs_frozen", (hipStream_t)stream, 0.0, (double)C * 48.0);
  hipLaunchKernelGGL(k_bn_bwd_coeffs_frozen, dim3((C + 7) / 8), dim3(256), 0, (hipStream_t)stream, C, sums, gamma, running_mean,
                     running_invstd, dgamma, dbeta, coef_abc);
  VK_CHECK_HIP(hipGetLastError());
  return VK_OK;
}

struct BnApplyArgs {
  size_t pixels; int C; const void* dy; const void* z; int mask_mode; const float* scale; const float* shift; const void* mask_src;
  const float* coef; const double* sums; double count; const float* gamma; const float* mean; const float* invstd; float* dgamma; float* dbeta;
  void* dz; void* g_out; int g_acc;
};

template <typename T>
static int launch_bn_bwd_apply(const BnApplyArgs& a, hipStream_t st) {
  const int CV = a.C / ElemTraits<T>::kVec;
  dim3 grid(grid_for(a.pixels * CV / 2 + 1)), block(256);
#define VK_APPLY(M) hipLaunchKernelGGL((k_bn_bwd_apply<T, M>), grid, block, 0, st, a.pixels, a.C, (const T*)a.dy, (const T*)a.z, a.scale, a.shift, \
    (const T*)a.mask_src, a.coef, a.sums, a.count, a.gamma, a.mean, a.invstd, a.dgamma, a.dbeta, (T*)a.dz, (T*)a.g_out, a.g_acc)
  if (a.mask_mode == 0) VK_APPLY(0);
  else if (a.mask_mode == 1) VK_APPLY(1);
  else VK_APPLY(2);
#undef VK_APPLY
  return VK_OK;
}

static int bn_bwd_apply_common(vk_dtype dtype, const BnApplyArgs& a, void* stream) {
  VK_CHECK_ARG(a.dy && a.z && a.dz && (a.coef || (a.sums && a.gamma && a.mean && a.invstd && a.dgamma && a.dbeta)), "vk_bn_bwd_apply: null argument");
  VK_CHECK_ARG(a.mask_mode >= 0 && a.mask_mode <= 2, "vk_bn_bwd_apply: mask_mode %d", a.mask_mode);
  VK_CHECK_ARG(a.mask_mode != 1 || (a.scale && a.shift), "vk_bn_bwd_apply: mask_mode 1 needs scale/shift");
  VK_CHECK_ARG(a.mask_mode != 2 || a.mask_src, "vk_bn_bwd_apply: mask_mode 2 needs mask_src");
  VK_CHECK_ARG(a.C <= 512 && a.C % 8 == 0, "vk_bn_bwd_apply: C=%d unsupported", a.C);
  hipStream_t st = (hipStream_t)stream;
  vkh::ProfScope ps_("bn_bwd_apply", st, 0.0, (double)a.pixels * a.C * (dtype == VK_F32 ? 4.0 : 2.0) * ((a.mask_mode == 2 ? 4.0 : 3.0) + (a.g_out ? (a.g_acc ? 2.0 : 1.0) : 0.0)));
  DISPATCH_T(dtype, launch_bn_bwd_apply<T>(a, st));
  VK_CHECK_HIP(hipGetLastError());
  return VK_OK;
}

extern "C" int vk_bn_bwd_apply(vk_dtype dtype, size_t pixels, int C, const void* dy, const void* z, int mask_mode,
                               const float* scale, const float* shift, const void* mask_src, const float* coef_abc, void* dz,
                               void* g_out, int g_accumulate, void* stream) {
  VK_CHECK_ARG(coef_abc, "vk_bn_bwd_apply: null coefficients");
  BnApplyArgs a{pixels, C, dy, z, mask_mode, scale, shift, mask_src, coef_abc, nullptr, 1.0, nullptr, nullptr, nullptr, nullptr, nullptr, dz, g_out, g_accumulate};
  return bn_bwd_apply_common(dtype, a, stream);
}

extern "C" int vk_bn_bwd_apply_fused(vk_dtype dtype, size_t pixels, int C, const void* dy, const void* z, int mask_mode,
                                     const float* scale, const float* shift, const void* mask_src, const double* sums, double count,
                                     const float* gamma, const float* save_mean, const float* save_invstd, float* dgamma, float* dbeta,
                                     void* dz, void* g_out, int g_accumulate, void* stream) {
  BnApplyArgs a{pixels, C, dy, z, mask_mode, scale, shift, mask_src, nullptr, sums, count, gamma, save_mean, save_invstd, dgamma, dbeta, dz, g_out, g_accumulate};
  return bn_bwd_apply_common(dtype, a, stream);
}

extern "C" int vk_upsample2x_bwd(vk_dtype dtype, int N, int H, int W, int C, const void* d_up, void* d_low, int accumulate,
                                 void* stream) {
  VK_CHECK_ARG(d_up && d_low && H % 2 == 0 && W % 2 == 0 && C % 8 == 0, "vk_upsample2x_bwd: bad argument");
  hipStream_t st = (hipStream_t)stream;
  vkh::ProfScope ps_("upsample2x_bwd", st, 0.0, (double)N * H * W * C * (dtype == VK_F32 ? 4.0 : 2.0) * 1.25);
  DISPATCH_T(dtype, hipLaunchKernelGGL(k_upsample2x_bwd<T>, dim3(grid_for((size_t)N * (H / 2) * (W / 2) * (C / ElemTraits<T>::kVec))),
                                       dim3(256), 0, st, N, H, W, C, (const T*)d_up, (T*)d_low, accumulate));
  VK_CHECK_HIP(hipGetLastError());
  return VK_OK;
}

extern "C" int vk_head_fwd(vk_dtype dtype, int N, int H, int W, const vk_src* src, const float* w9x16, const float* bias,
                           float* logits, void* stream) {
  VK_CHECK_ARG(src && src->ptr && w9x16 && bias && logits, "vk_head_fwd: null argument");
  VK_CHECK_ARG(src->C == 16 && !src->up, "vk_head_fwd: head input must have 16 channels, no upsample");
  hipStream_t st = (hipStream_t)stream;
  vkh::ProfScope ps_("head_fwd", st, 2.0 * 144.0 * N * H * W, (double)N * H * W * (16.0 * (dtype == VK_F32 ? 4.0 : 2.0) + 4.0));
  const int tx = (W + 15) / 16, ty = (H + 15) / 16;
  DISPATCH_T(dtype, hipLaunchKernelGGL(k_head_fwd<T>, dim3((unsigned)(N * tx * ty)), dim3(256), 0, st, N, H, W, tx, ty, (const T*)src->ptr,
                                       src->scale, src->shift, src->relu, w9x16, bias, logits));
  VK_CHECK_HIP(hipGetLastError());
  return VK_OK;
}

static int head_bwd_impl(vk_dtype dtype, int N, int H, int W, const vk_src* src, const float* w9x16, const float* dlogits,
                         void* dy, float* dw9x16, float* dbias, const vk_bnr* bnr, void* workspace, size_t workspace_bytes, void* stream);

extern "C" int vk_head_bwd(vk_dtype dtype, int N, int H, int W, const vk_src* src, const float* w9x16, const float* dlogits,
                           void* dy, float* dw9x16, float* dbias, void* workspace, size_t workspace_bytes, void* stream) {
  return head_bwd_impl(dtype, N, H, W, src, w9x16, dlogits, dy, dw9x16, dbias, nullptr, workspace, workspace_bytes, stream);
}

extern "C" int vk_head_bwd_fused(vk_dtype dtype, int N, int H, int W, const vk_src* src, const float* w9x16, const float* dlogits,
                                 void* dy, float* dw9x16, float* dbias, const vk_bnr* bnr, void* workspace, size_t workspace_bytes,
                                 void* stream) {
  VK_CHECK_ARG(bnr && bnr->z && bnr->scale && bnr->shift && bnr->sums, "vk_head_bwd_fused: incomplete vk_bnr");
  return head_bwd_impl(dtype, N, H, W, src, w9x16, dlogits, dy, dw9x16, dbias, bnr, workspace, workspace_bytes, stream);
}

static int head_bwd_impl(vk_dtype dtype, int N, int H, int W, const vk_src* src, const float* w9x16, const float* dlogits,
                         void* dy, float* dw9x16, float* dbias, const vk_bnr* bnr, void* workspace, size_t workspace_bytes, void* stream) {
  VK_CHECK_ARG(src && src->ptr && w9x16 && dlogits && dy && dw9x16 && dbias, "vk_head_bwd: null argument");
  VK_CHECK_ARG(src->C == 16 && !src->up, "vk_head_bwd: head input must have 16 channels, no upsample");
  hipStream_t st = (hipStream_t)stream;
  const int tx = (W + 15) / 16, ty = (H + 15) / 16;
  const int ntiles = N * tx * ty;
  const double eb = dtype == VK_F32 ? 4.0 : 2.0;
  if (dtype != VK_F32 && bnr && bnr->z == src->ptr && bnr->scale == src->scale && bnr->shift == src->shift && src->scale && src->shift &&
      !getenv("VK_HEAD_NO_MFMA")) {
    vkh::ProfScope ps_("head_bwd_mfma", st, 4.0 * 144.0 * N * H * W, (double)N * H * W * (32.0 * eb + 4.0));
    int nb = ntiles < 1024 ? ntiles : 1024;
    float* part = nullptr;
    if (workspace && workspace_bytes >= 148 * sizeof(float)) {
      const size_t cap = workspace_bytes / (148 * sizeof(float));
      if ((size_t)nb > cap) nb = (int)cap;
      part = (float*)workspace;
    }
    if (dtype == VK_BF16)
      hipLaunchKernelGGL(k_head_bwd_mfma<bf16_t>, dim3((unsigned)nb), dim3(256), 0, st, N, H, W, tx, ty, ntiles, (const bf16_t*)src->ptr, src->scale,
                         src->shift, src->relu, w9x16, dlogits, (bf16_t*)dy, bnr->sums, dw9x16, dbias, part);
    else
      hipLaunchKernelGGL(k_head_bwd_mfma<f16_t>, dim3((unsigned)nb), dim3(256), 0, st, N, H, W, tx, ty, ntiles, (const f16_t*)src->ptr, src->scale,
                         src->shift, src->relu, w9x16, dlogits, (f16_t*)dy, bnr->sums, dw9x16, dbias, part);
    if (part) hipLaunchKernelGGL(k_head_wgrad_reduce, dim3(10), dim3(256), 0, st, nb, (const float*)part, dw9x16, dbias);
    VK_CHECK_HIP(hipGetLastError());
    return VK_OK;
  }
  {
    vkh::ProfScope ps_("head_dgrad", st, 2.0 * 144.0 * N * H * W, (double)N * H * W * (16.0 * eb + 4.0));
    const int nbd = ntiles < 2048 ? ntiles : 2048;
    DISPATCH_T(dtype, hipLaunchKernelGGL(k_head_dgrad<T>, dim3((unsigned)nbd), dim3(256), 0, st, N, H, W, tx, ty, ntiles, w9x16, dlogits, (T*)dy,
                                         (const T*)(bnr ? bnr->z : nullptr), bnr ? bnr->scale : nullptr, bnr ? bnr->shift : nullptr,
                                         bnr ? bnr->sums : nullptr));
// ... 130 lines not shown
```

### vickers-hardness-unet_amd/csrc/engine.hip

```cpp
#include <stdarg.h>
#include <stdio.h>
#include <stdlib.h>
#include <string.h>

#include <algorithm>
#include <atomic>
#include <map>
#include <mutex>
#include <string>
#include <vector>

#include "vk_common.h"

namespace vkh {
static thread_local char g_err[512] = "";
void set_error(const char* fmt, ...) {
  va_list ap;
  va_start(ap, fmt);
  vsnprintf(g_err, sizeof(g_err), fmt, ap);
  va_end(ap);
}

struct ProfRec {
  std::string tag;
// ... 222 lines not shown
__global__ void k_cast_ranges(const CastRange* __restrict__ tab, const float* __restrict__ src, T* __restrict__ dst) {
  const CastRange r = tab[blockIdx.y];
  for (int64_t i = blockIdx.x * (int64_t)blockDim.x + threadIdx.x; i < r.count; i += (int64_t)gridDim.x * blockDim.x)
    st1(dst + r.begin + i, src[r.begin + i]);
}

template <typename T>
__global__ void k_pack_stem(const float* __restrict__ w, T* __restrict__ wp) {
  const int i = blockIdx.x * blockDim.x + threadIdx.x;
  if (i >= 64 * 7 * 32) return;
  const int j = i % 32, r = (i / 32) % 7, k = i / (32 * 7);
  const int s = j >> 2, c = j & 3;
  const float v = (s < 7 && c < 3) ? w[((k * 7 + r) * 7 + s) * 3 + c] : 0.f;
  st1(wp + i, v);
}

struct BnEvalEntry {
  int64_t g_off, b_off, rm_off, rv_off, out_off;
  int C, pad_;
};
__global__ void k_bn_eval_all(const BnEvalEntry* __restrict__ tab, const float* __restrict__ params, const float* __restrict__ bufs,
                              float* __restrict__ arena, float eps) {
  const BnEvalEntry e = tab[blockIdx.x];
  for (int c = threadIdx.x; c < e.C; c += blockDim.x) {
    const float invstd = (float)(1.0 / sqrt((double)bufs[e.rv_off + c] + (double)eps));
    const float sc = params[e.g_off + c] * invstd;
    arena[e.out_off + c] = sc;
    arena[e.out_off + e.C + c] = params[e.b_off + c] - bufs[e.rm_off + c] * sc;
  }
}

__global__ void k_inc_i64(int n, int64_t* p) {
  const int i = blockIdx.x * blockDim.x + threadIdx.x;
  if (i < n) p[i] += 1;
}

__global__ void k_inc_i64_masked(int n, int64_t* p, uint64_t frozen) {
  const int i = blockIdx.x * blockDim.x + threadIdx.x;
  if (i < n && !((frozen >> i) & 1ull)) p[i] += 1;
}

__global__ void k_bn_frozen_affine(const BnEvalEntry* __restrict__ tab, uint64_t frozen, const float* __restrict__ params,
                                   const float* __restrict__ bufs, float* __restrict__ arena, float eps) {
  if (!((frozen >> blockIdx.x) & 1ull)) return;
  const BnEvalEntry e = tab[blockIdx.x];
  float* f = arena + e.out_off;
  for (int c = threadIdx.x; c < e.C; c += blockDim.x) {
    const float invstd = (float)(1.0 / sqrt((double)bufs[e.rv_off + c] + (double)eps));
    const float sc = params[e.g_off + c] * invstd;
    f[c] = sc;
    f[e.C + c] = params[e.b_off + c] - bufs[e.rm_off + c] * sc;
    f[2 * e.C + c] = bufs[e.rm_off + c];
    f[3 * e.C + c] = invstd;
    f[4 * e.C + c] = sc;
    f[5 * e.C + c] = 0.f;
    f[6 * e.C + c] = 0.f;
  }
}

struct ConvL {
  std::string name;
  int Cin, K, R, stride, pad;
  int64_t w_off;
  int64_t wd_off;
  bool halo_fwd = false;
  bool halo_dg = false;
  int bn;
  int Hin, Hout;
  int Win, Wout;
  int w_t = -1, b_t = -1;
  int rank = 0;
  char* z = nullptr;
  char* g = nullptr;
};

struct BnL {
  std::string name;
  int C;
  int64_t g_off, b_off, rm_off, rv_off;
  int idx;
  int g_t = -1, b_t = -1;
  int rank = 0;
  double count;
  double* stats = nullptr;
  double* bsums = nullptr;
  float* scale = nullptr;
  float* shift = nullptr;
  float* mean = nullptr;
  float* invstd = nullptr;
  float* coef = nullptr;
  int64_t arena_off = 0;
};

struct BlockL {
  int conv1, conv2, convd;
  int Cin, C, stride, Hin, Hout, Win, Wout;
  bool in_has_grad_first;
  char* out = nullptr;
  char* gout = nullptr;
};

struct DecL {
  int conv1, conv2;
  int Cup, Cskip, Cout, H, W;
};

struct Act {
  const void* ptr;
  int C;
  const float* scale;
  const float* shift;
  int relu;
};

}

using namespace vk;

constexpr int kMaxStages = 16;
constexpr int kMaxBatch = 40;
constexpr size_t kEngineSlabBytes = 176u << 20;
constexpr size_t kGradScratchFloats = 2048;

struct vk_unet {
  vk_unet_config cfg;
  int classes = 1;
  int eb;
  std::vector<vk_tensor_info> infos;
  int n_ptensors = 0;
  std::vector<uint8_t> trainable;
  int last_rank = 0;
  uint64_t bn_frozen = 0, bn_frozen_fwd = 0;
  float* dx_in = nullptr;
  int input_rank = 0;
  unsigned mask_version = 0;
  std::vector<ConvL> convs;
  std::vector<BnL> bns;
  std::vector<BlockL> blocks;
  std::vector<DecL> decs;
  int stem_conv = -1, head_conv = -1;
  int layer_last_block[4];
  int64_t n_params = 0, n_bufs = 0, n_dgrad = 0;
  int64_t head_w_off = 0, head_b_off = 0;
  std::vector<std::pair<int64_t, int64_t>> buckets;
  size_t ws_bytes = 0;
  size_t off_x4 = 0, off_pool = 0, off_argmax = 0, off_gpool = 0, off_dup = 0, off_dlogits = 0, off_loss_sums = 0;
  size_t off_stats = 0, off_bsums = 0, stats_bytes = 0, off_farena = 0, farena_floats = 0, off_wf = 0, off_wd = 0, off_wstem = 0;
  size_t off_tab_pack = 0, off_tab_bn = 0, off_wslab = 0, off_wh = 0, off_tab_halo = 0, off_splitk = 0, splitk_bytes = 0;
  std::vector<HaloPackEntry> halo_tab;
  std::vector<size_t> off_z, off_g, off_out, off_gout;
  std::vector<char> g_prereduced;
  std::vector<char> tail_prereduced;
  float* params = nullptr;
  float* grads = nullptr;
  float* bufs = nullptr;
  int64_t* nbt = nullptr;
  char* ws = nullptr;
  bool bound = false;
  hipStream_t side = nullptr;
  hipEvent_t ev_fork = nullptr, ev_join = nullptr;
  bool side_dirty = false;
  struct WItem {
    vk_conv_desc d;
    const void* dz;
    float* dw;
  };
  struct WPlan {
    bool built = false;
    int target = 0, n = 0;
    unsigned version = 0;
    vk::WgradBatchPlan plan;
  };
  std::vector<WItem> pending;
  WPlan wplans[kMaxStages][2];
  size_t off_tab_wbatch = 0;
  std::vector<PackEntry> pack_tab;
  std::vector<CastRange> cast_tab;
  size_t off_tab_cast = 0;
  size_t off_gscratch = 0;
  size_t off_mloss = 0, mloss_bytes = 0;
  std::vector<BnEvalEntry> bn_tab;
  std::map<std::string, std::pair<void*, std::vector<int>>> debug;

  int N() const { return cfg.N; }
};

namespace {

size_t align_up(size_t v, size_t a) { return (v + a - 1) / a * a; }

bool need_from(const vk_unet* h, int rank) { return h->last_rank >= rank; }
bool trains(const vk_unet* h, int t) { return h->trainable[(size_t)t] != 0; }
bool frozen(const vk_unet* h, const BnL& b) { return (h->bn_frozen_fwd >> b.idx) & 1ull; }
bool bn_sums_needed(const vk_unet* h, const BnL& b) { return !frozen(h, b) || trains(h, b.g_t) || trains(h, b.b_t); }
float* grad_or_sink(vk_unet* h, int t, int64_t off, int sink_off) {
  return trains(h, t) ? h->grads + off : (float*)(h->ws + h->off_gscratch) + sink_off;
}
float* dgamma_of(vk_unet* h, const BnL& b) { return grad_or_sink(h, b.g_t, b.g_off, 0); }
float* dbeta_of(vk_unet* h, const BnL& b) { return grad_or_sink(h, b.b_t, b.b_off, 512); }

int add_info(vk_unet* h, const std::string& name, int kind, std::vector<int> dims, int64_t offset, int64_t numel) {
  vk_tensor_info ti;
  memset(&ti, 0, sizeof(ti));
  snprintf(ti.name, sizeof(ti.name), "%s", name.c_str());
  ti.kind = kind;
  ti.ndim = (int)dims.size();
  for (size_t i = 0; i < dims.size() && i < 4; ++i) ti.dims[i] = dims[i];
  ti.offset = offset;
  ti.numel = numel;
  h->infos.push_back(ti);
  return kind <= 1 ? h->n_ptensors++ : -1;
}

int add_conv(vk_unet* h, const std::string& name, int Cin, int K, int R, int stride, int pad, int Hin, int Win, bool bias = false) {
  ConvL c;
  c.name = name;
  c.Cin = Cin; c.K = K; c.R = R; c.stride = stride; c.pad = pad;
  c.Hin = Hin; c.Win = Win;
  c.Hout = (Hin + 2 * pad - R) / stride + 1;
  c.Wout = (Win + 2 * pad - R) / stride + 1;
  c.w_off = h->n_params;
  c.wd_off = -1;
  c.bn = -1;
  const int64_t numel = (int64_t)K * Cin * R * R;
  c.w_t = add_info(h, name + ".weight", 0, {K, Cin, R, R}, c.w_off, numel);
  h->n_params += (int64_t)align_up((size_t)numel, 4);
  if (bias) {
    c.b_t = add_info(h, name + ".bias", 1, {K}, h->n_params, K);
    h->n_params += (int64_t)align_up((size_t)K, 4);
  }
  h->convs.push_back(c);
  return (int)h->convs.size() - 1;
}

int add_bn(vk_unet* h, const std::string& name, int C, double count) {
  BnL b;
  b.name = name;
  b.C = C;
  b.count = count;
  b.idx = (int)h->bns.size();
  b.g_off = h->n_params;
  b.g_t = add_info(h, name + ".weight", 1, {C}, b.g_off, C);
  h->n_params += C;
  b.b_off = h->n_params;
  b.b_t = add_info(h, name + ".bias", 1, {C}, b.b_off, C);
  h->n_params += C;
  b.rm_off = h->n_bufs;
  add_info(h, name + ".running_mean", 2, {C}, b.rm_off, C);
  h->n_bufs += C;
  b.rv_off = h->n_bufs;
  add_info(h, name + ".running_var", 2, {C}, b.rv_off, C);
  h->n_bufs += C;
  add_info(h, name + ".num_batches_tracked", 3, {}, b.idx, 1);
  h->bns.push_back(b);
  return b.idx;
}

void build_topology(vk_unet* h) {
  const int S = h->cfg.size, SW = h->cfg.width, N = h->cfg.N;
  auto cnt = [&](int Hres, int Wres) { return (double)N * Hres * Wres; };
  h->stem_conv = add_conv(h, "encoder.conv1", 3, 64, 7, 2, 3, S, SW);
  h->convs[h->stem_conv].bn = add_bn(h, "encoder.bn1", 64, cnt(S / 2, SW / 2));
  const int nblocks[4] = {3, 4, 6, 3};
  const int planes[4] = {64, 128, 256, 512};
  int inpl = 64, res = S / 4, resw = SW / 4;
  std::vector<int64_t> layer_start(4), layer3_mid(1);
  std::vector<int64_t> block_start;
  for (int L = 0; L < 4; ++L) {
    layer_start[L] = h->n_params;
    for (int b = 0; b < nblocks[L]; ++b) {
      block_start.push_back(h->n_params);
      const int stride = (b == 0 && L > 0) ? 2 : 1;
      const std::string pre = "encoder.layer" + std::to_string(L + 1) + "." + std::to_string(b);
      BlockL blk;
      blk.Cin = inpl; blk.C = planes[L]; blk.stride = stride; blk.Hin = res; blk.Hout = res / stride; blk.Win = resw; blk.Wout = resw / stride;
      blk.conv1 = add_conv(h, pre + ".conv1", inpl, planes[L], 3, stride, 1, res, resw);
      h->convs[blk.conv1].bn = add_bn(h, pre + ".bn1", planes[L], cnt(blk.Hout, blk.Wout));
      blk.conv2 = add_conv(h, pre + ".conv2", planes[L], planes[L], 3, 1, 1, blk.Hout, blk.Wout);
      h->convs[blk.conv2].bn = add_bn(h, pre + ".bn2", planes[L], cnt(blk.Hout, blk.Wout));
      blk.convd = -1;
      if (stride != 1 || inpl != planes[L]) {
        blk.convd = add_conv(h, pre + ".downsample.0", inpl, planes[L], 1, stride, 0, res, resw);
        h->convs[blk.convd].bn = add_bn(h, pre + ".downsample.1", planes[L], cnt(blk.Hout, blk.Wout));
      }
      blk.in_has_grad_first = (b == 0 && L > 0);
      h->blocks.push_back(blk);
      inpl = planes[L];
      res = blk.Hout;
      resw = blk.Wout;
    }
    h->layer_last_block[L] = (int)h->blocks.size() - 1;
  }
  const int dec_in[5] = {512, 256, 128, 64, 32};
  const int dec_skip[5] = {256, 128, 64, 64, 0};
  const int dec_out[5] = {256, 128, 64, 32, 16};
  std::vector<int64_t> dec_start(5);
  int dres = S / 32, dresw = SW / 32;
  for (int i = 0; i < 5; ++i) {
    dec_start[i] = h->n_params;
    dres *= 2;
    dresw *= 2;
    const std::string pre = "decoder.blocks." + std::to_string(i);
    DecL d;
    d.Cup = dec_in[i]; d.Cskip = dec_skip[i]; d.Cout = dec_out[i]; d.H = dres; d.W = dresw;
    d.conv1 = add_conv(h, pre + ".conv1.0", dec_in[i] + dec_skip[i], dec_out[i], 3, 1, 1, dres, dresw);
    h->convs[d.conv1].bn = add_bn(h, pre + ".conv1.1", dec_out[i], cnt(dres, dresw));
    d.conv2 = add_conv(h, pre + ".conv2.0", dec_out[i], dec_out[i], 3, 1, 1, dres, dresw);
    h->convs[d.conv2].bn = add_bn(h, pre + ".conv2.1", dec_out[i], cnt(dres, dresw));
    h->decs.push_back(d);
  }
  const int64_t head_start = h->n_params;
  (void)head_start;
  h->head_conv = add_conv(h, "segmentation_head.0", 16, h->classes, 3, 1, 1, S, SW, true);
  h->head_w_off = h->convs[h->head_conv].w_off;
  h->head_b_off = h->head_w_off + (int64_t)align_up((size_t)144 * h->classes, 4);
  h->n_params = (int64_t)align_up((size_t)h->n_params, 64);
  for (size_t i = 0; i < h->convs.size(); ++i) {
    if ((int)i == h->stem_conv || (int)i == h->head_conv) continue;
    ConvL& c = h->convs[i];
    c.wd_off = h->n_dgrad;
    h->n_dgrad += (int64_t)align_up((size_t)c.K * c.Cin * c.R * c.R, 8);
  }
// ... 517 lines not shown
    if (k.convd >= 0) {
      ConvL& cd = h->convs[k.convd];
      RET_IF(run_conv(h, cd, to_src(cur), null_src(), training, st));
      const BnL& bd = h->bns[cd.bn];
      RET_IF(vk_bn_add_relu(dt, pixels, k.C, c2.z, b2.scale, b2.shift, cd.z, bd.scale, bd.shift, k.out, st));
    } else {
      RET_IF(vk_bn_add_relu(dt, pixels, k.C, c2.z, b2.scale, b2.shift, cur.ptr, nullptr, nullptr, k.out, st));
    }
    cur = Act{k.out, k.C, nullptr, nullptr, 0};
  }
  Act skips[5];
  skips[0] = Act{h->blocks[h->layer_last_block[2]].out, 256, nullptr, nullptr, 0};
  skips[1] = Act{h->blocks[h->layer_last_block[1]].out, 128, nullptr, nullptr, 0};
  skips[2] = Act{h->blocks[h->layer_last_block[0]].out, 64, nullptr, nullptr, 0};
  skips[3] = bn_act(h, stem);
  skips[4] = Act{nullptr, 0, nullptr, nullptr, 0};
  Act xd = cur;
  for (size_t i = 0; i < h->decs.size(); ++i) {
    DecL& d = h->decs[i];
    ConvL& c1 = h->convs[d.conv1];
    ConvL& c2 = h->convs[d.conv2];
    const bool small_plan = (size_t)N * S * SW <= 4u * 512 * 512;
    if (!training && h->classes == 1 && i + 1 == h->decs.size() && dt != VK_F32 && !d.Cskip && d.Cup == 32 && c1.K == 16 && c2.K == 16 && c1.halo_fwd &&
        !c2.halo_fwd && S % 16 == 0 && SW % 16 == 0 && !getenv("VK_NO_TAIL_FUSION") && (small_plan || getenv("VK_TAIL_FUSION"))) {
      const vk_src s0 = to_src(xd, 1);
      const BnL& b1 = h->bns[c1.bn];
      const BnL& b2 = h->bns[c2.bn];
      return vk_dec4_tail_eval(dt, N, S, SW, &s0, fwd_weights(h, c1), b1.scale, b1.shift, fwd_weights(h, c2), b2.scale, b2.shift,
                               h->params + h->head_w_off, h->params + h->head_b_off, logits, st);
    }
    RET_IF(run_conv(h, c1, to_src(xd, 1), d.Cskip ? to_src(skips[i]) : null_src(), training, st));
    RET_IF(run_conv(h, c2, to_src(bn_act(h, c1)), null_src(), training, st));
    xd = bn_act(h, c2);
  }
  vk_src hs = to_src(xd);
  if (h->classes == 1) RET_IF(vk_head_fwd(dt, N, S, SW, &hs, h->params + h->head_w_off, h->params + h->head_b_off, logits, st));
  else RET_IF(vk_head_fwd_multi(dt, N, S, SW, h->classes, &hs, h->params + h->head_w_off, h->params + h->head_b_off, logits, st));
  if (training) {
    if (h->bn_frozen_fwd) hipLaunchKernelGGL(k_inc_i64_masked, dim3(1), dim3(64), 0, st, (int)h->bns.size(), h->nbt, h->bn_frozen_fwd);
    else hipLaunchKernelGGL(k_inc_i64, dim3(1), dim3(64), 0, st, (int)h->bns.size(), h->nbt);
    VK_CHECK_HIP(hipGetLastError());
  }
  return VK_OK;
}

extern "C" int vk_unet_loss_ex(vk_unet* h, int mode, const void* logits, const void* target, float* loss_out, float grad_scale,
                               float w_ce, float w_dice, void* stream) {
  VK_CHECK_ARG(h && h->bound && logits && target && loss_out, "vk_unet_loss_ex: plan not bound or null tensor");
  VK_CHECK_ARG(mode == VK_LOSS_BINARY || mode == VK_LOSS_MULTILABEL || mode == VK_LOSS_MULTICLASS, "vk_unet_loss_ex: bad mode %d", mode);
  VK_CHECK_ARG(mode != VK_LOSS_BINARY || h->classes == 1, "vk_unet_loss_ex: the binary loss needs classes == 1 (the plan has %d)", h->classes);
  VK_CHECK_ARG(mode != VK_LOSS_MULTICLASS || h->classes >= 2, "vk_unet_loss_ex: the multi-class loss needs classes >= 2");
  if (h->classes == 1) return vk_unet_loss(h, (const float*)logits, (const float*)target, loss_out, grad_scale, w_ce, w_dice, stream);
  const int N = h->cfg.N, HW = h->cfg.size * h->cfg.width;
  float* dl = h->cfg.training ? (float*)(h->ws + h->off_dlogits) : nullptr;
  if (mode == VK_LOSS_MULTILABEL)
    return vk_multilabel_loss(N, h->classes, HW, (const float*)logits, (const float*)target, h->ws + h->off_mloss, h->mloss_bytes, loss_out,
                              dl, grad_scale, w_ce, w_dice, stream);
  return vk_multiclass_loss(N, h->classes, HW, (const float*)logits, (const int64_t*)target, h->ws + h->off_mloss, h->mloss_bytes, loss_out,
                            dl, grad_scale, w_ce, w_dice, stream);
}

extern "C" int vk_unet_loss(vk_unet* h, const float* logits, const float* target, float* loss_out, float grad_scale, float w_bce,
                            float w_dice, void* stream) {
  VK_CHECK_ARG(h && h->bound && logits && target && loss_out, "vk_unet_loss: plan not bound or null tensor");
  VK_CHECK_ARG(h->classes == 1, "vk_unet_loss: the binary loss needs classes == 1; use vk_unet_loss_ex");
  const size_t count = (size_t)h->cfg.N * h->cfg.size * h->cfg.width;
  float* dl = h->cfg.training ? (float*)(h->ws + h->off_dlogits) : nullptr;
  return vk_bce_dice_loss(count, logits, target, (double*)(h->ws + h->off_loss_sums), loss_out, dl, grad_scale, w_bce, w_dice, stream);
}

#ifndef VK_BN_APPLY_FUSED_MAXC_DEFAULT
#define VK_BN_APPLY_FUSED_MAXC_DEFAULT 0
#endif
namespace {

int bn_bwd_phase2(vk_unet* h, BnL& b, int C, size_t pixels, const void* dy, const void* z, int mask_mode, const void* mask_src, void* dz,
                  void* g_out, int g_acc, hipStream_t st) {
  static const int maxc = getenv("VK_BN_APPLY_FUSED_MAXC") ? atoi(getenv("VK_BN_APPLY_FUSED_MAXC")) : VK_BN_APPLY_FUSED_MAXC_DEFAULT;
  if (frozen(h, b)) {
    if (trains(h, b.g_t) || trains(h, b.b_t))
      RET_IF(vk_bn_bwd_coeffs_frozen(C, b.bsums, h->params + b.g_off, b.mean, b.invstd, dgamma_of(h, b), dbeta_of(h, b), b.coef, st));
    return vk_bn_bwd_apply(h->cfg.dtype, pixels, C, dy, z, mask_mode, b.scale, b.shift, mask_src, b.coef, dz, g_out, g_acc, st);
  }
  if (C <= maxc)
    return vk_bn_bwd_apply_fused(h->cfg.dtype, pixels, C, dy, z, mask_mode, b.scale, b.shift, mask_src, b.bsums, b.count, h->params + b.g_off,
                                 b.mean, b.invstd, dgamma_of(h, b), dbeta_of(h, b), dz, g_out, g_acc, st);
  RET_IF(vk_bn_bwd_coeffs(C, b.bsums, b.count, h->params + b.g_off, b.mean, b.invstd, dgamma_of(h, b), dbeta_of(h, b), b.coef, st));
  return vk_bn_bwd_apply(h->cfg.dtype, pixels, C, dy, z, mask_mode, b.scale, b.shift, mask_src, b.coef, dz, g_out, g_acc, st);
}

int bn_relu_bwd_inplace(vk_unet* h, ConvL& c, bool prereduced, hipStream_t st) {
  BnL& b = h->bns[c.bn];
  const size_t pixels = (size_t)h->cfg.N * c.Hout * c.Wout;
  if (!prereduced && bn_sums_needed(h, b)) RET_IF(vk_bn_bwd_reduce(h->cfg.dtype, pixels, c.K, c.g, c.z, 1, b.scale, b.shift, nullptr, b.bsums, st));
  return bn_bwd_phase2(h, b, c.K, pixels, c.g, c.z, prereduced ? 0 : 1, nullptr, c.g, nullptr, 0, st);
}

int wgrad_stream(vk_unet* h, hipStream_t st, hipStream_t* out) {
  *out = st;
  if (!h->side) return VK_OK;
  VK_CHECK_HIP(hipEventRecord(h->ev_fork, st));
  VK_CHECK_HIP(hipStreamWaitEvent(h->side, h->ev_fork, 0));
  h->side_dirty = true;
  *out = h->side;
  return VK_OK;
}

int join_side(vk_unet* h, hipStream_t st) {
  if (!h->side || !h->side_dirty) return VK_OK;
  VK_CHECK_HIP(hipEventRecord(h->ev_join, h->side));
  VK_CHECK_HIP(hipStreamWaitEvent(st, h->ev_join, 0));
  h->side_dirty = false;
  return VK_OK;
}

int conv_wgrad(vk_unet* h, ConvL& c, const vk_src& s0, const vk_src& s1, hipStream_t st) {
  vk_conv_desc d = conv_desc(h, c, s0, s1);
  if (!h->side && vk::wgrad_batch_supports(&d)) {
    h->pending.push_back(vk_unet::WItem{d, c.g, h->grads + c.w_off});
    return VK_OK;
  }
  hipStream_t ws;
  RET_IF(wgrad_stream(h, st, &ws));
  return vk_conv_wgrad(&d, c.g, h->grads + c.w_off, h->ws + h->off_wslab, VK_WGRAD_WORKSPACE_BYTES, ws);
}

vk_bnr bnr_of(vk_unet* h, ConvL& target) {
  BnL& b = h->bns[target.bn];
  vk_bnr r;
  r.z = target.z; r.scale = b.scale; r.shift = b.shift; r.sums = b.bsums; r.mask = nullptr; r.accumulate = 0;
  return r;
}

vk_conv_desc dgrad_desc(vk_unet* h, ConvL& c) {
  vk_conv_desc d;
  d.dtype = h->cfg.dtype;
  d.N = h->cfg.N; d.H = c.Hout; d.W = c.Wout; d.Ho = c.Hin; d.Wo = c.Win;
  d.K = c.Cin; d.R = c.R; d.S = c.R; d.stride = c.stride; d.pad = c.pad; d.transposed = 1;
  vk_src s;
  s.ptr = c.g; s.C = c.K; s.up = 0; s.scale = nullptr; s.shift = nullptr; s.relu = 0;
  d.src0 = s;
  d.src1 = null_src();
  return d;
}

int conv_dgrad_into(vk_unet* h, ConvL& c, ConvL& into, bool* fused, hipStream_t st) {
  vk_conv_desc d = dgrad_desc(h, c);
  vk_bnr r = bnr_of(h, into);
  int rc = getenv("VK_NO_BNR_FUSION") ? VK_ERR_UNSUPPORTED : vk_conv_dgrad_fused(&d, dgrad_weights(h, c), into.g, nullptr, 0, 0, &r, st);
  *fused = rc == VK_OK;
  if (rc != VK_ERR_UNSUPPORTED) return rc;
  if (c.halo_dg) return vk_conv_fwd_packed(&d, dgrad_weights(h, c), into.g, nullptr, 0, 0, nullptr, st);
  return vk_conv_fwd(&d, dgrad_weights(h, c), into.g, nullptr, 0, 0, nullptr, st);
}

int conv_dgrad(vk_unet* h, ConvL& c, void* y, void* y1, int split, int accumulate, hipStream_t st) {
  vk_conv_desc d;
  d.dtype = h->cfg.dtype;
  d.N = h->cfg.N; d.H = c.Hout; d.W = c.Wout; d.Ho = c.Hin; d.Wo = c.Win;
  d.K = c.Cin; d.R = c.R; d.S = c.R; d.stride = c.stride; d.pad = c.pad; d.transposed = 1;
  vk_src s;
  s.ptr = c.g; s.C = c.K; s.up = 0; s.scale = nullptr; s.shift = nullptr; s.relu = 0;
  d.src0 = s;
  d.src1 = null_src();
  if (c.halo_dg) return vk_conv_fwd_packed(&d, dgrad_weights(h, c), y, y1, split, accumulate, nullptr, st);
  return vk_conv_fwd(&d, dgrad_weights(h, c), y, y1, split, accumulate, nullptr, st);
}

int backward_decoder(vk_unet* h, int i, hipStream_t st) {
  DecL& d = h->decs[i];
  ConvL& c1 = h->convs[d.conv1];
  ConvL& c2 = h->convs[d.conv2];
  const int N = h->cfg.N;
  ConvL& stem = h->convs[h->stem_conv];
  Act xprev, skip{nullptr, 0, nullptr, nullptr, 0};
  void* g_prev;
  if (i == 0) {
    BlockL& f5 = h->blocks[h->layer_last_block[3]];
    xprev = Act{f5.out, 512, nullptr, nullptr, 0};
    g_prev = f5.gout;
  } else {
    ConvL& pc2 = h->convs[h->decs[i - 1].conv2];
    xprev = bn_act(h, pc2);
    g_prev = pc2.g;
  }
  void* g_skip = nullptr;
  if (i <= 2) {
    BlockL& fb = h->blocks[h->layer_last_block[2 - i]];
    skip = Act{fb.out, fb.C, nullptr, nullptr, 0};
    g_skip = fb.gout;
  } else if (i == 3) {
    skip = bn_act(h, stem);
    g_skip = stem.g;
  }
  const BnL& bn1 = h->bns[c1.bn];
  if (!need_from(h, h->bns[c2.bn].rank)) {
    if (i > 0) h->g_prereduced[h->decs[i - 1].conv2] = 0;
    return VK_OK;
  }
  RET_IF(bn_relu_bwd_inplace(h, c2, h->g_prereduced[d.conv2] != 0, st));
  const bool into1 = need_from(h, bn1.rank);
  bool fused1 = false;
  if (into1) RET_IF(conv_dgrad_into(h, c2, c1, &fused1, st));
  if (trains(h, c2.w_t)) RET_IF(conv_wgrad(h, c2, to_src(bn_act(h, c1)), null_src(), st));
  if (i > 0) h->g_prereduced[h->decs[i - 1].conv2] = 0;
  if (!into1) return VK_OK;
  RET_IF(bn_relu_bwd_inplace(h, c1, fused1, st));
  if (need_from(h, c1.rank + 1)) {
    vk_conv_desc dd = dgrad_desc(h, c1);
    vk_bnr r;
    const bool want_bnr = i > 0 && !getenv("VK_NO_BNR_FUSION");
    if (want_bnr) r = bnr_of(h, h->convs[h->decs[i - 1].conv2]);
    const int rc = vk_conv_dgrad_fused(&dd, dgrad_weights(h, c1), g_prev, d.Cskip ? g_skip : nullptr, d.Cskip ? d.Cup : 0, 1,
                                       want_bnr ? &r : nullptr, st);
    if (rc == VK_OK && want_bnr) h->g_prereduced[h->decs[i - 1].conv2] = 1;
    if (rc != VK_OK && rc != VK_ERR_UNSUPPORTED) return rc;
    if (rc == VK_ERR_UNSUPPORTED) {
      void* dup = h->ws + h->off_dup;
      if (d.Cskip) RET_IF(conv_dgrad(h, c1, dup, g_skip, d.Cup, 0, st));
      else RET_IF(conv_dgrad(h, c1, dup, nullptr, 0, 0, st));
      RET_IF(vk_upsample2x_bwd(h->cfg.dtype, N, d.H, d.W, d.Cup, dup, g_prev, 0, st));
    }
  }
  if (!trains(h, c1.w_t)) return VK_OK;
  return conv_wgrad(h, c1, to_src(xprev, 1), d.Cskip ? to_src(skip) : null_src(), st);
}

int backward_block(vk_unet* h, int bi, hipStream_t st) {
  BlockL& k = h->blocks[bi];
  ConvL& c1 = h->convs[k.conv1];
  ConvL& c2 = h->convs[k.conv2];
  BnL& b2 = h->bns[c2.bn];
  const vk_dtype dt = h->cfg.dtype;
  const size_t pixels = (size_t)h->cfg.N * k.Hout * k.Wout;
  if (!need_from(h, b2.rank)) {
    h->tail_prereduced[(size_t)bi] = 0;
    return VK_OK;
  }
  Act xin;
  void* gin;
  if (bi == 0) {
    xin = Act{h->ws + h->off_pool, 64, nullptr, nullptr, 0};
    gin = h->ws + h->off_gpool;
  } else {
    BlockL& pb = h->blocks[bi - 1];
    xin = Act{pb.out, pb.C, nullptr, nullptr, 0};
    gin = pb.gout;
  }
  const bool pre = h->tail_prereduced[(size_t)bi] != 0;
  h->tail_prereduced[(size_t)bi] = 0;
  if (bi > 0) h->tail_prereduced[(size_t)bi - 1] = 0;
  const int mm = pre ? 0 : 2;
  if (!pre && bn_sums_needed(h, b2)) RET_IF(vk_bn_bwd_reduce(dt, pixels, k.C, k.gout, c2.z, 2, nullptr, nullptr, k.out, b2.bsums, st));
  if (k.convd < 0) {
    RET_IF(bn_bwd_phase2(h, b2, k.C, pixels, k.gout, c2.z, mm, k.out, c2.g, gin, k.in_has_grad_first ? 1 : 0, st));
  } else {
    ConvL& cd = h->convs[k.convd];
    BnL& bd = h->bns[cd.bn];
    RET_IF(bn_bwd_phase2(h, b2, k.C, pixels, k.gout, c2.z, mm, k.out, c2.g, nullptr, 0, st));
    if (bn_sums_needed(h, bd)) RET_IF(vk_bn_bwd_reduce(dt, pixels, k.C, k.gout, cd.z, mm, nullptr, nullptr, k.out, bd.bsums, st));
    RET_IF(bn_bwd_phase2(h, bd, k.C, pixels, k.gout, cd.z, mm, k.out, cd.g, nullptr, 0, st));
  }
  const bool into1 = need_from(h, h->bns[c1.bn].rank);
  bool fused1 = false;
  if (into1) RET_IF(conv_dgrad_into(h, c2, c1, &fused1, st));
  if (trains(h, c2.w_t)) RET_IF(conv_wgrad(h, c2, to_src(bn_act(h, c1)), null_src(), st));
  if (!into1) return k.convd >= 0 && trains(h, h->convs[k.convd].w_t) ? conv_wgrad(h, h->convs[k.convd], to_src(xin), null_src(), st) : VK_OK;
  RET_IF(bn_relu_bwd_inplace(h, c1, fused1, st));
  const bool into_gin = need_from(h, c1.rank + 1);
  bool tail_fused = false;
  const int tail_maxc = getenv("VK_TAIL_BNR_MAXC") ? atoi(getenv("VK_TAIL_BNR_MAXC")) : 1 << 20;
  if (into_gin && k.convd < 0 && bi > 0 && c1.halo_dg && k.C <= tail_maxc && !getenv("VK_NO_TAIL_BNR_FUSION")) {
    BlockL& pb = h->blocks[bi - 1];
    ConvL& pc2 = h->convs[pb.conv2];
    vk_conv_desc dd = dgrad_desc(h, c1);
    vk_bnr r;
    r.z = pc2.z; r.scale = nullptr; r.shift = nullptr; r.sums = h->bns[pc2.bn].bsums; r.mask = pb.out; r.accumulate = 1;
    const int rc = vk_conv_dgrad_fused(&dd, dgrad_weights(h, c1), gin, nullptr, 0, 0, &r, st);
    if (rc == VK_OK) { tail_fused = true; h->tail_prereduced[(size_t)bi - 1] = 1; }
    else if (rc != VK_ERR_UNSUPPORTED) return rc;
  }
  if (into_gin && !tail_fused) RET_IF(conv_dgrad(h, c1, gin, nullptr, 0, 1, st));
  if (k.convd >= 0) {
    ConvL& cd = h->convs[k.convd];
    if (into_gin) RET_IF(conv_dgrad(h, cd, gin, nullptr, 0, 1, st));
    if (trains(h, c1.w_t)) RET_IF(conv_wgrad(h, c1, to_src(xin), null_src(), st));
    return trains(h, cd.w_t) ? conv_wgrad(h, cd, to_src(xin), null_src(), st) : VK_OK;
  }
  return trains(h, c1.w_t) ? conv_wgrad(h, c1, to_src(xin), null_src(), st) : VK_OK;
}

int stem_coeffs(vk_unet* h, BnL& b, hipStream_t st) {
  if (!frozen(h, b))
    return vk_bn_bwd_coeffs(64, b.bsums, b.count, h->params + b.g_off, b.mean, b.invstd, dgamma_of(h, b), dbeta_of(h, b), b.coef, st);
  if (!trains(h, b.g_t) && !trains(h, b.b_t)) return VK_OK;
  return vk_bn_bwd_coeffs_frozen(64, b.bsums, h->params + b.g_off, b.mean, b.invstd, dgamma_of(h, b), dbeta_of(h, b), b.coef, st);
}

int backward_stem(vk_unet* h, hipStream_t st) {
  const int N = h->cfg.N, S = h->cfg.size, SW = h->cfg.width;
  ConvL& stem = h->convs[h->stem_conv];
  if (!need_from(h, h->bns[stem.bn].rank)) return VK_OK;
  BnL& b = h->bns[stem.bn];
  const bool want_w = trains(h, stem.w_t);
  const float* const w = h->params + stem.w_off;
  if (getenv("VK_NO_POOL_BNR_FUSION")) {
    RET_IF(vk_maxpool_bwd(h->cfg.dtype, N, S / 2, SW / 2, 64, h->ws + h->off_gpool, (const uint8_t*)(h->ws + h->off_argmax), stem.g, st));
    RET_IF(bn_relu_bwd_inplace(h, stem, false, st));
  } else {
    RET_IF(vk_maxpool_bwd_bn_reduce(h->cfg.dtype, N, S / 2, SW / 2, 64, h->ws + h->off_gpool, (const uint8_t*)(h->ws + h->off_argmax), stem.z,
                                    b.scale, b.shift, stem.g, b.bsums, st));
    if (!want_w && !h->dx_in) return stem_coeffs(h, b, st);
    if (h->cfg.dtype != VK_F32 && !getenv("VK_NO_STEM_BNA")) {
      RET_IF(stem_coeffs(h, b, st));
      int rc = VK_OK;
      if (want_w) {
        hipStream_t ws;
        RET_IF(wgrad_stream(h, st, &ws));
        rc = vk_stem_wgrad_bn(h->cfg.dtype, N, S, SW, h->ws + h->off_x4, stem.g, stem.z, b.coef, h->grads + stem.w_off,
                              h->ws + h->off_wslab, VK_WGRAD_WORKSPACE_BYTES, ws);
        if (rc != VK_OK && rc != VK_ERR_UNSUPPORTED) return rc;
      }
      if (rc == VK_OK) return h->dx_in ? vk_stem_dgrad(h->cfg.dtype, N, S, SW, stem.g, stem.z, b.coef, w, h->dx_in, st) : VK_OK;
      RET_IF(vk_bn_bwd_apply(h->cfg.dtype, (size_t)N * (S / 2) * (SW / 2), 64, stem.g, stem.z, 0, b.scale, b.shift, nullptr, b.coef, stem.g, nullptr, 0, st));
    } else {
      RET_IF(bn_relu_bwd_inplace(h, stem, true, st));
    }
  }
  if (want_w) {
    hipStream_t ws;
    RET_IF(wgrad_stream(h, st, &ws));
    RET_IF(vk_stem_wgrad(h->cfg.dtype, N, S, SW, h->ws + h->off_x4, stem.g, h->grads + stem.w_off, h->ws + h->off_wslab, VK_WGRAD_WORKSPACE_BYTES, ws));
  }
  return h->dx_in ? vk_stem_dgrad(h->cfg.dtype, N, S, SW, stem.g, nullptr, nullptr, w, h->dx_in, st) : VK_OK;
}

int flush_wgrads(vk_unet* h, int stage, hipStream_t st) {
  const int n = (int)h->pending.size();
  if (n == 0) return VK_OK;
  char* const slab = h->ws + h->off_wslab;
  auto each = [&]() {
    int rc = VK_OK;
    for (const vk_unet::WItem& it : h->pending) {
      rc = vk_conv_wgrad(&it.d, it.dz, it.dw, slab, kEngineSlabBytes, st);
      if (rc != VK_OK) break;
    }
    h->pending.clear();
    return rc;
  };
  if (n == 1 || n > kMaxBatch || stage < 0 || stage >= kMaxStages) return each();
  const int target = 256 - vkh::reserved_cus();
  const int slot = target == 256 ? 0 : 1;
  vk_unet::WPlan& wp = h->wplans[stage][slot];
  char* const tables = h->ws + h->off_tab_wbatch + ((size_t)stage * 2 + slot) * VK_WGRAD_BATCH_TABLE_BYTES;
  if (!wp.built || wp.target != target || wp.n != n || wp.version != h->mask_version) {
    if (wp.built) VK_CHECK_HIP(hipStreamSynchronize(st));
    vk_conv_desc descs[kMaxBatch];
    const void* dz[kMaxBatch];
    float* dw[kMaxBatch];
    for (int i = 0; i < n; ++i) { descs[i] = h->pending[(size_t)i].d; dz[i] = h->pending[(size_t)i].dz; dw[i] = h->pending[(size_t)i].dw; }
// ... 80 lines not shown
```

### vickers-hardness-unet_amd/csrc/vk_common.h

```cpp
#pragma once
#include <hip/hip_runtime.h>
#include <stdint.h>

#include "../../include/vk_unet.h"

namespace vk {

struct bf16_t { uint16_t v; };
struct f16_t  { uint16_t v; };

typedef __attribute__((ext_vector_type(8))) __bf16   bf16x8_t;
typedef __attribute__((ext_vector_type(8))) _Float16 f16x8_t;
typedef __attribute__((ext_vector_type(4))) float    f32x4_t;
typedef __attribute__((ext_vector_type(4))) uint32_t u32x4_t;
typedef __attribute__((ext_vector_type(2))) uint32_t u32x2_t;
typedef __attribute__((ext_vector_type(4))) short    s16x4_t;
typedef __attribute__((ext_vector_type(2))) float    f32x2_t;
typedef __attribute__((ext_vector_type(2))) __bf16   bf16x2_t;
typedef __attribute__((ext_vector_type(2))) _Float16 f16x2_t;
typedef __attribute__((ext_vector_type(2))) short    s16x2_t;

template <typename T> struct ElemTraits;
template <> struct ElemTraits<float> {
  static constexpr int kBytes = 4;
// ... 166 lines not shown
};

__device__ __forceinline__ __amdgpu_buffer_rsrc_t make_rsrc(const void* p, uint32_t bytes) {
  return __builtin_amdgcn_make_buffer_rsrc(const_cast<void*>(p), 0, bytes, 0x00020000);
}
__device__ __forceinline__ u32x4_t buf_load16(__amdgpu_buffer_rsrc_t r, uint32_t byte_off) {
  return __builtin_amdgcn_raw_buffer_load_b128(r, byte_off, 0, 0);
}
static constexpr uint32_t kOOB = 0x80000000u;

typedef __attribute__((ext_vector_type(4))) int i32x4_t;
__device__ __forceinline__ i32x4_t make_rsrc_words(const void* p, uint32_t bytes) {
  const uint64_t a = (uint64_t)p;
  i32x4_t r;
  r[0] = __builtin_amdgcn_readfirstlane((int)(uint32_t)a);
  r[1] = __builtin_amdgcn_readfirstlane((int)(uint32_t)(a >> 32));
  r[2] = __builtin_amdgcn_readfirstlane((int)bytes);
  r[3] = 0x00020000;
  return r;
}
__device__ __forceinline__ void lds_dma16_hidden(i32x4_t srd, uint32_t byte_off, uint32_t lds_addr) {
  unsigned keep;
  asm volatile("s_nop 4\n\ts_mov_b32 %0, m0\n\ts_mov_b32 m0, %3\n\ts_nop 0\n\tbuffer_load_dwordx4 %1, %2, 0 offen lds\n\ts_mov_b32 m0, %0"
               : "=&s"(keep)
               : "v"(byte_off), "s"(srd), "s"(lds_addr)
               : "memory");
}
__device__ __forceinline__ void lds_dma_wait_all() { asm volatile("s_waitcnt vmcnt(0)" ::: "memory"); }

struct FastDiv {
  uint32_t mul, shr, div;
};
__device__ __forceinline__ uint32_t fdiv(uint32_t n, FastDiv d) { return d.div == 1 ? n : (__umulhi(n, d.mul) >> d.shr); }

template <int CTRL, int ROW_MASK = 0xF>
__device__ __forceinline__ float dpp_f(float v) {
  return __builtin_bit_cast(float, __builtin_amdgcn_update_dpp(0, __builtin_bit_cast(int, v), CTRL, ROW_MASK, 0xF, false));
}
__device__ __forceinline__ float row16_sum(float v) {
  v += dpp_f<0xB1>(v);
  v += dpp_f<0x4E>(v);
  v += dpp_f<0x141>(v);
  v += dpp_f<0x140>(v);
  return v;
}
__device__ __forceinline__ float wave_sum(float v) {
  v = row16_sum(v);
  v += dpp_f<0x142, 0xA>(v);
  v += dpp_f<0x143, 0xC>(v);
  return __builtin_bit_cast(float, __builtin_amdgcn_readlane(__builtin_bit_cast(int, v), 63));
}
__device__ __forceinline__ double wave_sum_d(double v) {
#pragma unroll
  for (int o = 32; o > 0; o >>= 1) v += __shfl_xor(v, o, 64);
  return v;
}

}

namespace vkh {
inline vk::FastDiv make_fastdiv(uint32_t d) {
  vk::FastDiv f;
  f.div = d;
  if (d <= 1) { f.mul = 0; f.shr = 0; f.div = 1; return f; }
  uint32_t lg = 0;
  while ((1u << lg) < d) ++lg;
  uint32_t p = 31 + lg;
  f.mul = (uint32_t)(((1ull << p) + d - 1) / d);
  f.shr = p - 32;
  return f;
}
void set_error(const char* fmt, ...);
int reserved_cus();

struct ProfScope {
  int idx;
  hipStream_t st;
  hipEvent_t ev_end;
  ProfScope(const char* tag, hipStream_t stream, double flops, double bytes);
  ~ProfScope();
};
}

#define VK_CHECK_ARG(cond, ...)                \
  do {                                         \
    if (!(cond)) {                             \
      vkh::set_error(__VA_ARGS__);             \
      return VK_ERR_ARG;                       \
    }                                          \
  } while (0)

#define VK_CHECK_HIP(expr)                                                              \
  do {                                                                                  \
    hipError_t e_ = (expr);                                                             \
    if (e_ != hipSuccess) {                                                             \
      vkh::set_error("%s failed: %s (%s:%d)", #expr, hipGetErrorString(e_), __FILE__, __LINE__); \
      return (int)e_;                                                                   \
    }                                                                                   \
  } while (0)

namespace vk {
struct WgradBatchPlan {
  int nwg = 0, nsegs = 0, ntred = 0, nlayers = 0;
  size_t off_layers = 0, off_segs = 0, off_wgfirst = 0, off_tred = 0, slab_need = 0;
  double flops = 0.0, bytes = 0.0;
};
bool wgrad_batch_supports(const vk_conv_desc* d);
int wgrad_batch_build(const vk_conv_desc* descs, const void* const* dz, float* const* dw, int n, int target_blocks, void* tables,
                      size_t tables_bytes, WgradBatchPlan* plan);
int wgrad_batch_launch(vk_dtype dt, const WgradBatchPlan& plan, const void* tables, void* slab, size_t slab_bytes, hipStream_t st);
}
```

Before: 2997.

## Use fewer BN stat replicas for wide channels and fold coeffs into backward apply

Adds a runtime replica count for BN-statistics atomics. Wide-channel BN layers (C>=128, bf16/f16 training) use min(32, 2048/C) replicas instead of 32, which shrinks the replica reduction. For those layers the backward apply kernel computes the BN backward coefficients from the replica sums in each block, with block 0 updating dgamma/dbeta, and prefetches its first batch of dy/z/mask loads before that work. This removes the separate coefficient kernel launch and part of the reduction cost, but it raises atomic contention on fewer replicas and repeats the coefficient math in every block.

```diff
diff --git a/vickers-hardness-unet_amd/csrc/conv_halo.hip b/vickers-hardness-unet_amd/csrc/conv_halo.hip
--- a/vickers-hardness-unet_amd/csrc/conv_halo.hip
+++ b/vickers-hardness-unet_amd/csrc/conv_halo.hip
@@ -59,6 +59,7 @@
   const float* bnr_shift;
   double* bnr_sums;
   const void* bnr_mask;
+  int repl;
 };
 
 template <typename T, int TH, int BN, int WGM, int WGN>
@@ -298,12 +299,12 @@
       } else if (p.bnr_sums) {
         const int kc = p.ld0;
         if (n0 + tid < kc) {
-          double* sp = p.bnr_sums + (size_t)(blockIdx.x % VK_STATS_REPLICAS) * 2 * kc;
+          double* sp = p.bnr_sums + (size_t)(blockIdx.x % p.repl) * 2 * kc;
           atomicAdd(sp + n0 + tid, (double)a);
           atomicAdd(sp + kc + n0 + tid, (double)b);
         }
       } else {
-        double* sp = p.stats + (size_t)(blockIdx.x % VK_STATS_REPLICAS) * 2 * p.K;
+        double* sp = p.stats + (size_t)(blockIdx.x % p.repl) * 2 * p.K;
         atomicAdd(sp + n0 + tid, (double)a);
         atomicAdd(sp + p.K + n0 + tid, (double)b);
       }
@@ -318,12 +319,12 @@
     if (p.bnr_sums) {
       const int kc = p.ld0;
       if (n0 + tid < kc) {
-        double* sp = p.bnr_sums + (size_t)(blockIdx.x % VK_STATS_REPLICAS) * 2 * kc;
+        double* sp = p.bnr_sums + (size_t)(blockIdx.x % p.repl) * 2 * kc;
         atomicAdd(sp + n0 + tid, d[0]);
         atomicAdd(sp + kc + n0 + tid, d[1]);
       }
     } else if (p.stats) {
-      double* sp = p.stats + (size_t)(blockIdx.x % VK_STATS_REPLICAS) * 2 * p.K;
+      double* sp = p.stats + (size_t)(blockIdx.x % p.repl) * 2 * p.K;
       atomicAdd(sp + n0 + tid, d[0]);
       atomicAdd(sp + p.K + n0 + tid, d[1]);
     }
@@ -1755,6 +1756,7 @@
   p.y0 = y;
   p.ld0 = 64;
   p.stats = stats;
+  p.repl = stats_replicas();
   p.N = N; p.H = H / 2; p.W = W / 2; p.K = 64; p.C = 4;
   p.Hi = H; p.Wi = W;
   p.tiles_x = (p.W + 15) / 16;
@@ -2183,7 +2185,7 @@
   }
 
   if (want_sums) {
-    double* const sp = (p.bnr_sums ? p.bnr_sums : p.stats) + (size_t)(strip % VK_STATS_REPLICAS) * 2 * ld;
+    double* const sp = (p.bnr_sums ? p.bnr_sums : p.stats) + (size_t)(strip % p.repl) * 2 * ld;
 #pragma unroll
     for (int a = 0; a < TC; ++a)
 #pragma unroll
@@ -2752,6 +2754,7 @@
   p.bnr_shift = bnr ? bnr->shift : nullptr;
   p.bnr_sums = bnr ? bnr->sums : nullptr;
   p.bnr_mask = bnr ? bnr->mask : nullptr;
+  p.repl = stats_replicas();
   p.nchunks = c16 ? 1 : C / ck;
   if (p.bnr_mask && (c16 || s2 || s2d || pool2)) return VK_ERR_UNSUPPORTED;
   if (eb == 2 && !s2 && !s2d && !p.bnr_mask && (c16 || C == 32)) {
diff --git a/vickers-hardness-unet_amd/csrc/elementwise.hip b/vickers-hardness-unet_amd/csrc/elementwise.hip
--- a/vickers-hardness-unet_amd/csrc/elementwise.hip
+++ b/vickers-hardness-unet_amd/csrc/elementwise.hip
@@ -10,6 +10,13 @@
   if (b < 1) b = 1;
   return (int)b;
 }
+
+constexpr int kBnFoldMaxBlocks = 512;
+
+static thread_local int g_stats_repl = VK_STATS_REPLICAS;
+int stats_replicas() { return g_stats_repl; }
+StatsReplicaScope::StatsReplicaScope(int r) : prev(g_stats_repl) { g_stats_repl = r; }
+StatsReplicaScope::~StatsReplicaScope() { g_stats_repl = prev; }
 
 template <typename T>
 __global__ void k_input_transform(int N, int H, int W, const float* __restrict__ x, T* __restrict__ x4) {
@@ -322,28 +329,35 @@
 }
 
 template <typename T, int MASK>
-__device__ __forceinline__ void masked_grad(const T* dy, const T* z, const T* mask_src, size_t off, const float* sc,
-                                            const float* sh, float* g, float* zf) {
+__device__ __forceinline__ void masked_grad_raw(const u32x4_t& rdy, const u32x4_t& rz, const u32x4_t& rm, const float* sc, const float* sh,
+                                                float* g, float* zf) {
   constexpr int VE = ElemTraits<T>::kVec;
-  Vec16<T>::unpack(*reinterpret_cast<const u32x4_t*>(dy + off), g);
-  Vec16<T>::unpack(*reinterpret_cast<const u32x4_t*>(z + off), zf);
+  Vec16<T>::unpack(rdy, g);
+  Vec16<T>::unpack(rz, zf);
   if (MASK == 1) {
 #pragma unroll
     for (int j = 0; j < VE; ++j)
       if (!(fmaf(zf[j], sc[j], sh[j]) > 0.f)) g[j] = 0.f;
   } else if (MASK == 2) {
     float m[VE];
-    Vec16<T>::unpack(*reinterpret_cast<const u32x4_t*>(mask_src + off), m);
+    Vec16<T>::unpack(rm, m);
 #pragma unroll
     for (int j = 0; j < VE; ++j)
       if (!(m[j] > 0.f)) g[j] = 0.f;
   }
+}
+
+template <typename T, int MASK>
+__device__ __forceinline__ void masked_grad(const T* dy, const T* z, const T* mask_src, size_t off, const float* sc,
+                                            const float* sh, float* g, float* zf) {
+  const u32x4_t rm = MASK == 2 ? *reinterpret_cast<const u32x4_t*>(mask_src + off) : u32x4_t{0u, 0u, 0u, 0u};
+  masked_grad_raw<T, MASK>(*reinterpret_cast<const u32x4_t*>(dy + off), *reinterpret_cast<const u32x4_t*>(z + off), rm, sc, sh, g, zf);
 }
 
 template <typename T, int MASK>
 __global__ __launch_bounds__(256) void k_bn_bwd_reduce(size_t pixels, int C, const T* __restrict__ dy, const T* __restrict__ z,
                                                        const float* __restrict__ scale, const float* __restrict__ shift,
-                                                       const T* __restrict__ mask_src, double* sums) {
+                                                       const T* __restrict__ mask_src, double* sums, int repl) {
   constexpr int VE = ElemTraits<T>::kVec;
   const int CV = C / VE;
   const int rows = 256 / CV;
@@ -392,10 +406,56 @@
       a += red[(t * VE + cj) * 2];
       b += red[(t * VE + cj) * 2 + 1];
     }
-    double* sp = sums + (size_t)(blockIdx.x % VK_STATS_REPLICAS) * 2 * C;
+    double* sp = sums + (size_t)(blockIdx.x % repl) * 2 * C;
     atomicAdd(sp + c, a);
     atomicAdd(sp + C + c, b);
   }
+}
+
+__device__ __forceinline__ void bn_replica_sum(const double* __restrict__ sums, int C, int c, int R, double& s1, double& s2) {
+  double a[VK_STATS_REPLICAS], b[VK_STATS_REPLICAS];
+#pragma unroll
+  for (int q = 0; q < VK_STATS_REPLICAS; ++q)
+    if (q < R) {
+      a[q] = sums[(size_t)q * 2 * C + c];
+      b[q] = sums[(size_t)q * 2 * C + C + c];
+    }
+  s1 = a[0];
+  s2 = b[0];
+#pragma unroll
+  for (int q = 1; q < VK_STATS_REPLICAS; ++q)
+    if (q < R) {
+      s1 += a[q];
+      s2 += b[q];
+    }
+}
+
+struct BnBwdCoef {
+  float dg, db, a, b, c;
+};
+__device__ __forceinline__ BnBwdCoef bn_bwd_coef(double sg, double sgz, double count, float save_mean, float save_invstd, float gamma) {
+  const double mu = save_mean, r = save_invstd, ga = gamma;
+  const double dg = r * (sgz - mu * sg);
+  const double db = sg;
+  const double a = ga * r;
+  const double b = -ga * r * r * dg / count;
+  const double cc = -a * db / count - b * mu;
+  return BnBwdCoef{(float)dg, (float)db, (float)a, (float)b, (float)cc};
+}
+
+__global__ __launch_bounds__(256) void k_bn_bwd_coeffs_r(int C, int R, const double* __restrict__ sums, double count,
+                                                         const float* __restrict__ gamma, const float* __restrict__ save_mean,
+                                                         const float* __restrict__ save_invstd, float* dgamma, float* dbeta, float* coef) {
+  const int c = blockIdx.x * blockDim.x + threadIdx.x;
+  if (c >= C) return;
+  double sg, sgz;
+  bn_replica_sum(sums, C, c, R, sg, sgz);
+  const BnBwdCoef k = bn_bwd_coef(sg, sgz, count, save_mean[c], save_invstd[c], gamma[c]);
+  dgamma[c] += k.dg;
+  dbeta[c] += k.db;
+  coef[c] = k.a;
+  coef[C + c] = k.b;
+  coef[2 * C + c] = k.c;
 }
 
 __global__ __launch_bounds__(256) void k_bn_bwd_coeffs(int C, const double* __restrict__ sums, double count, const float* __restrict__ gamma,
@@ -453,26 +513,52 @@
   coef[2 * C + c] = 0.f;
 }
 
-template <typename T, int MASK>
+template <typename T, int MASK, bool FOLD = false>
 __global__ __launch_bounds__(256) void k_bn_bwd_apply(size_t pixels, int C, const T* __restrict__ dy, const T* __restrict__ z,
                                                       const float* __restrict__ scale, const float* __restrict__ shift, const T* __restrict__ mask_src,
                                                       const float* __restrict__ coef, const double* __restrict__ sums, double count,
                                                       const float* __restrict__ gamma, const float* __restrict__ save_mean,
                                                       const float* __restrict__ save_invstd, float* dgamma, float* dbeta, T* __restrict__ dz, T* g_out,
-                                                      int g_acc) {
+                                                      int g_acc, int repl) {
   constexpr int VE = ElemTraits<T>::kVec;
-  constexpr int U = 2;
+  constexpr int U = FOLD ? 4 : 2;
   const int CV = C / VE;
   const size_t total = pixels * CV;
   const size_t stride = (size_t)gridDim.x * blockDim.x;
   const size_t t0 = blockIdx.x * (size_t)blockDim.x + threadIdx.x;
   const int c0 = (int)(t0 % CV) * VE;
+  u32x4_t pdy[U], pz[U], pm[U];
+  if constexpr (FOLD) {
+#pragma unroll
+    for (int u = 0; u < U; ++u) {
+      const size_t k = t0 + u * stride;
+      pm[u] = u32x4_t{0u, 0u, 0u, 0u};
+      if (k < total) {
+        pdy[u] = *reinterpret_cast<const u32x4_t*>(dy + k * VE);
+        pz[u] = *reinterpret_cast<const u32x4_t*>(z + k * VE);
+        if (MASK == 2) pm[u] = *reinterpret_cast<const u32x4_t*>(mask_src + k * VE);
+      }
+    }
+  }
   __shared__ float cf[3][512];
   if (coef) {
     for (int c = threadIdx.x; c < C; c += blockDim.x) {
       cf[0][c] = coef[c];
       cf[1][c] = coef[C + c];
       cf[2][c] = coef[2 * C + c];
+    }
+  } else if (FOLD) {
+    for (int c = threadIdx.x; c < C; c += blockDim.x) {
+      double sg, sgz;
+      bn_replica_sum(sums, C, c, repl, sg, sgz);
+      const BnBwdCoef k = bn_bwd_coef(sg, sgz, count, save_mean[c], save_invstd[c], gamma[c]);
+      cf[0][c] = k.a;
+      cf[1][c] = k.b;
+      cf[2][c] = k.c;
+      if (blockIdx.x == 0) {
+        dgamma[c] += k.dg;
+        dbeta[c] += k.db;
+      }
     }
   } else {
     static_assert(VK_STATS_REPLICAS == 32, "replica mapping");
@@ -515,7 +601,35 @@
     cb[j] = cf[1][c0 + j];
     cc[j] = cf[2][c0 + j];
   }
-  for (size_t i = t0; i < total; i += U * stride) {
+  auto emit = [&](size_t k, float* g, const float* zf) {
+    float o[VE];
+#pragma unroll
+    for (int j = 0; j < VE; ++j) o[j] = fmaf(ca[j], g[j], fmaf(cb[j], zf[j], cc[j]));
+    *reinterpret_cast<u32x4_t*>(dz + k * VE) = Vec16<T>::pack(o);
+    if (g_out) {
+      u32x4_t* gp = reinterpret_cast<u32x4_t*>(g_out + k * VE);
+      if (g_acc) {
+        float old[VE];
+        Vec16<T>::unpack(*gp, old);
+#pragma unroll
+        for (int j = 0; j < VE; ++j) g[j] += old[j];
+      }
+      *gp = Vec16<T>::pack(g);
+    }
+  };
+  size_t i0 = t0;
+  if constexpr (FOLD) {
+#pragma unroll
+    for (int u = 0; u < U; ++u) {
+      const size_t k = t0 + u * stride;
+      if (k >= total) continue;
+      float g[VE], zf[VE];
+      masked_grad_raw<T, MASK>(pdy[u], pz[u], pm[u], sc, sh, g, zf);
+      emit(k, g, zf);
+    }
+    i0 += U * stride;
+  }
+  for (size_t i = i0; i < total; i += U * stride) {
     float g[U][VE], zf[U][VE];
 #pragma unroll
     for (int u = 0; u < U; ++u)
@@ -524,20 +638,7 @@
     for (int u = 0; u < U; ++u) {
       const size_t k = i + u * stride;
       if (k >= total) continue;
-      float o[VE];
-#pragma unroll
-      for (int j = 0; j < VE; ++j) o[j] = fmaf(ca[j], g[u][j], fmaf(cb[j], zf[u][j], cc[j]));
-      *reinterpret_cast<u32x4_t*>(dz + k * VE) = Vec16<T>::pack(o);
-      if (g_out) {
-        u32x4_t* gp = reinterpret_cast<u32x4_t*>(g_out + k * VE);
-        if (g_acc) {
-          float old[VE];
-          Vec16<T>::unpack(*gp, old);
-#pragma unroll
-          for (int j = 0; j < VE; ++j) g[u][j] += old[j];
-        }
-        *gp = Vec16<T>::pack(g[u]);
-      }
+      emit(k, g[u], zf[u]);
     }
   }
 }
@@ -1323,9 +1424,10 @@
   if (nb > 2048) nb = 2048;
   if (nb < 1) nb = 1;
   dim3 grid((unsigned)nb), block(256);
-  if (mask_mode == 0) hipLaunchKernelGGL((k_bn_bwd_reduce<T, 0>), grid, block, 0, st, pixels, C, (const T*)dy, (const T*)z, scale, shift, (const T*)mask_src, sums);
-  else if (mask_mode == 1) hipLaunchKernelGGL((k_bn_bwd_reduce<T, 1>), grid, block, 0, st, pixels, C, (const T*)dy, (const T*)z, scale, shift, (const T*)mask_src, sums);
-  else hipLaunchKernelGGL((k_bn_bwd_reduce<T, 2>), grid, block, 0, st, pixels, C, (const T*)dy, (const T*)z, scale, shift, (const T*)mask_src, sums);
+  const int R = stats_replicas();
+  if (mask_mode == 0) hipLaunchKernelGGL((k_bn_bwd_reduce<T, 0>), grid, block, 0, st, pixels, C, (const T*)dy, (const T*)z, scale, shift, (const T*)mask_src, sums, R);
+  else if (mask_mode == 1) hipLaunchKernelGGL((k_bn_bwd_reduce<T, 1>), grid, block, 0, st, pixels, C, (const T*)dy, (const T*)z, scale, shift, (const T*)mask_src, sums, R);
+  else hipLaunchKernelGGL((k_bn_bwd_reduce<T, 2>), grid, block, 0, st, pixels, C, (const T*)dy, (const T*)z, scale, shift, (const T*)mask_src, sums, R);
   return VK_OK;
 }
 
@@ -1367,17 +1469,25 @@
   size_t pixels; int C; const void* dy; const void* z; int mask_mode; const float* scale; const float* shift; const void* mask_src;
   const float* coef; const double* sums; double count; const float* gamma; const float* mean; const float* invstd; float* dgamma; float* dbeta;
   void* dz; void* g_out; int g_acc;
+  int repl = 0;
 };
 
 template <typename T>
 static int launch_bn_bwd_apply(const BnApplyArgs& a, hipStream_t st) {
   const int CV = a.C / ElemTraits<T>::kVec;
   dim3 grid(grid_for(a.pixels * CV / 2 + 1)), block(256);
-#define VK_APPLY(M) hipLaunchKernelGGL((k_bn_bwd_apply<T, M>), grid, block, 0, st, a.pixels, a.C, (const T*)a.dy, (const T*)a.z, a.scale, a.shift, \
-    (const T*)a.mask_src, a.coef, a.sums, a.count, a.gamma, a.mean, a.invstd, a.dgamma, a.dbeta, (T*)a.dz, (T*)a.g_out, a.g_acc)
-  if (a.mask_mode == 0) VK_APPLY(0);
-  else if (a.mask_mode == 1) VK_APPLY(1);
-  else VK_APPLY(2);
+#define VK_APPLY(M, F) hipLaunchKernelGGL((k_bn_bwd_apply<T, M, F>), grid, block, 0, st, a.pixels, a.C, (const T*)a.dy, (const T*)a.z, a.scale, \
+    a.shift, (const T*)a.mask_src, a.coef, a.sums, a.count, a.gamma, a.mean, a.invstd, a.dgamma, a.dbeta, (T*)a.dz, (T*)a.g_out, a.g_acc, a.repl)
+  if (a.repl > 0) {
+    grid = dim3(grid_for(a.pixels * CV / 4 + 1, 256, kBnFoldMaxBlocks));
+    if (a.mask_mode == 0) VK_APPLY(0, true);
+    else if (a.mask_mode == 1) VK_APPLY(1, true);
+    else VK_APPLY(2, true);
+    return VK_OK;
+  }
+  if (a.mask_mode == 0) VK_APPLY(0, false);
+  else if (a.mask_mode == 1) VK_APPLY(1, false);
+  else VK_APPLY(2, false);
 #undef VK_APPLY
   return VK_OK;
 }
@@ -1401,6 +1511,29 @@
   VK_CHECK_ARG(coef_abc, "vk_bn_bwd_apply: null coefficients");
   BnApplyArgs a{pixels, C, dy, z, mask_mode, scale, shift, mask_src, coef_abc, nullptr, 1.0, nullptr, nullptr, nullptr, nullptr, nullptr, dz, g_out, g_accumulate};
   return bn_bwd_apply_common(dtype, a, stream);
+}
+
+namespace vk {
+int bn_bwd_coeffs_r(int C, int R, const double* sums, double count, const float* gamma, const float* save_mean, const float* save_invstd,
+                    float* dgamma, float* dbeta, float* coef_abc, hipStream_t st) {
+  VK_CHECK_ARG(C > 0 && R > 0 && R <= VK_STATS_REPLICAS && sums && gamma && save_mean && save_invstd && dgamma && dbeta && coef_abc,
+               "bn_bwd_coeffs_r: bad argument");
+  vkh::ProfScope ps_("bn_bwd_coeffs", st, 0.0, (double)C * (16.0 * R + 20.0));
+  hipLaunchKernelGGL(k_bn_bwd_coeffs_r, dim3((C + 63) / 64), dim3(64), 0, st, C, R, sums, count, gamma, save_mean, save_invstd, dgamma,
+                     dbeta, coef_abc);
+  VK_CHECK_HIP(hipGetLastError());
+  return VK_OK;
+}
+
+int bn_bwd_apply_fold_r(vk_dtype dtype, size_t pixels, int C, int R, const void* dy, const void* z, int mask_mode, const float* scale,
+                        const float* shift, const void* mask_src, const double* sums, double count, const float* gamma,
+                        const float* save_mean, const float* save_invstd, float* dgamma, float* dbeta, void* dz, void* g_out, int g_acc,
+                        hipStream_t st) {
+  VK_CHECK_ARG(dtype != VK_F32 && R > 0 && R <= VK_STATS_REPLICAS, "bn_bwd_apply_fold_r: dtype %d, R=%d", (int)dtype, R);
+  BnApplyArgs a{pixels, C, dy, z, mask_mode, scale, shift, mask_src, nullptr, sums, count, gamma, save_mean, save_invstd, dgamma, dbeta, dz, g_out, g_acc};
+  a.repl = R;
+  return bn_bwd_apply_common(dtype, a, st);
+}
 }
 
 extern "C" int vk_bn_bwd_apply_fused(vk_dtype dtype, size_t pixels, int C, const void* dy, const void* z, int mask_mode,
diff --git a/vickers-hardness-unet_amd/csrc/engine.hip b/vickers-hardness-unet_amd/csrc/engine.hip
--- a/vickers-hardness-unet_amd/csrc/engine.hip
+++ b/vickers-hardness-unet_amd/csrc/engine.hip
@@ -328,6 +328,7 @@
   int g_t = -1, b_t = -1;
   int rank = 0;
   double count;
+  int repl = VK_STATS_REPLICAS;
   double* stats = nullptr;
   double* bsums = nullptr;
   float* scale = nullptr;
@@ -439,6 +440,7 @@
 bool trains(const vk_unet* h, int t) { return h->trainable[(size_t)t] != 0; }
 bool frozen(const vk_unet* h, const BnL& b) { return (h->bn_frozen_fwd >> b.idx) & 1ull; }
 bool bn_sums_needed(const vk_unet* h, const BnL& b) { return !frozen(h, b) || trains(h, b.g_t) || trains(h, b.b_t); }
+int bwd_repl(const vk_unet* h, const BnL& b) { return frozen(h, b) ? VK_STATS_REPLICAS : b.repl; }
 float* grad_or_sink(vk_unet* h, int t, int64_t off, int sink_off) {
   return trains(h, t) ? h->grads + off : (float*)(h->ws + h->off_gscratch) + sink_off;
 }
@@ -484,6 +486,7 @@
   b.name = name;
   b.C = C;
   b.count = count;
+  if (h->cfg.training && h->cfg.dtype != VK_F32 && C >= 128) b.repl = std::min(VK_STATS_REPLICAS, 2048 / C);
   b.idx = (int)h->bns.size();
   b.g_off = h->n_params;
   b.g_t = add_info(h, name + ".weight", 1, {C}, b.g_off, C);
@@ -1167,6 +1170,13 @@
       RET_IF(vk_bn_bwd_coeffs_frozen(C, b.bsums, h->params + b.g_off, b.mean, b.invstd, dgamma_of(h, b), dbeta_of(h, b), b.coef, st));
     return vk_bn_bwd_apply(h->cfg.dtype, pixels, C, dy, z, mask_mode, b.scale, b.shift, mask_src, b.coef, dz, g_out, g_acc, st);
   }
+  if (b.repl < VK_STATS_REPLICAS) {
+    if (!getenv("VK_NO_BN_FOLD_BWD"))
+      return vk::bn_bwd_apply_fold_r(h->cfg.dtype, pixels, C, b.repl, dy, z, mask_mode, b.scale, b.shift, mask_src, b.bsums, b.count,
+                                     h->params + b.g_off, b.mean, b.invstd, dgamma_of(h, b), dbeta_of(h, b), dz, g_out, g_acc, st);
+    RET_IF(vk::bn_bwd_coeffs_r(C, b.repl, b.bsums, b.count, h->params + b.g_off, b.mean, b.invstd, dgamma_of(h, b), dbeta_of(h, b), b.coef, st));
+    return vk_bn_bwd_apply(h->cfg.dtype, pixels, C, dy, z, mask_mode, b.scale, b.shift, mask_src, b.coef, dz, g_out, g_acc, st);
+  }
   if (C <= maxc)
     return vk_bn_bwd_apply_fused(h->cfg.dtype, pixels, C, dy, z, mask_mode, b.scale, b.shift, mask_src, b.bsums, b.count, h->params + b.g_off,
                                  b.mean, b.invstd, dgamma_of(h, b), dbeta_of(h, b), dz, g_out, g_acc, st);
@@ -1177,7 +1187,10 @@
 int bn_relu_bwd_inplace(vk_unet* h, ConvL& c, bool prereduced, hipStream_t st) {
   BnL& b = h->bns[c.bn];
   const size_t pixels = (size_t)h->cfg.N * c.Hout * c.Wout;
-  if (!prereduced && bn_sums_needed(h, b)) RET_IF(vk_bn_bwd_reduce(h->cfg.dtype, pixels, c.K, c.g, c.z, 1, b.scale, b.shift, nullptr, b.bsums, st));
+  if (!prereduced && bn_sums_needed(h, b)) {
+    vk::StatsReplicaScope rs_(bwd_repl(h, b));
+    RET_IF(vk_bn_bwd_reduce(h->cfg.dtype, pixels, c.K, c.g, c.z, 1, b.scale, b.shift, nullptr, b.bsums, st));
+  }
   return bn_bwd_phase2(h, b, c.K, pixels, c.g, c.z, prereduced ? 0 : 1, nullptr, c.g, nullptr, 0, st);
 }
 
@@ -1232,7 +1245,11 @@
 int conv_dgrad_into(vk_unet* h, ConvL& c, ConvL& into, bool* fused, hipStream_t st) {
   vk_conv_desc d = dgrad_desc(h, c);
   vk_bnr r = bnr_of(h, into);
-  int rc = getenv("VK_NO_BNR_FUSION") ? VK_ERR_UNSUPPORTED : vk_conv_dgrad_fused(&d, dgrad_weights(h, c), into.g, nullptr, 0, 0, &r, st);
+  int rc;
+  {
+    vk::StatsReplicaScope rs_(bwd_repl(h, h->bns[into.bn]));
+    rc = getenv("VK_NO_BNR_FUSION") ? VK_ERR_UNSUPPORTED : vk_conv_dgrad_fused(&d, dgrad_weights(h, c), into.g, nullptr, 0, 0, &r, st);
+  }
   *fused = rc == VK_OK;
   if (rc != VK_ERR_UNSUPPORTED) return rc;
   if (c.halo_dg) return vk_conv_fwd_packed(&d, dgrad_weights(h, c), into.g, nullptr, 0, 0, nullptr, st);
@@ -1296,6 +1313,7 @@
     vk_bnr r;
     const bool want_bnr = i > 0 && !getenv("VK_NO_BNR_FUSION");
     if (want_bnr) r = bnr_of(h, h->convs[h->decs[i - 1].conv2]);
+    vk::StatsReplicaScope rs_(want_bnr ? bwd_repl(h, h->bns[h->convs[h->decs[i - 1].conv2].bn]) : VK_STATS_REPLICAS);
     const int rc = vk_conv_dgrad_fused(&dd, dgrad_weights(h, c1), g_prev, d.Cskip ? g_skip : nullptr, d.Cskip ? d.Cup : 0, 1,
                                        want_bnr ? &r : nullptr, st);
     if (rc == VK_OK && want_bnr) h->g_prereduced[h->decs[i - 1].conv2] = 1;
@@ -1336,14 +1354,20 @@
   h->tail_prereduced[(size_t)bi] = 0;
   if (bi > 0) h->tail_prereduced[(size_t)bi - 1] = 0;
   const int mm = pre ? 0 : 2;
-  if (!pre && bn_sums_needed(h, b2)) RET_IF(vk_bn_bwd_reduce(dt, pixels, k.C, k.gout, c2.z, 2, nullptr, nullptr, k.out, b2.bsums, st));
+  if (!pre && bn_sums_needed(h, b2)) {
+    vk::StatsReplicaScope rs_(bwd_repl(h, b2));
+    RET_IF(vk_bn_bwd_reduce(dt, pixels, k.C, k.gout, c2.z, 2, nullptr, nullptr, k.out, b2.bsums, st));
+  }
   if (k.convd < 0) {
     RET_IF(bn_bwd_phase2(h, b2, k.C, pixels, k.gout, c2.z, mm, k.out, c2.g, gin, k.in_has_grad_first ? 1 : 0, st));
   } else {
     ConvL& cd = h->convs[k.convd];
     BnL& bd = h->bns[cd.bn];
     RET_IF(bn_bwd_phase2(h, b2, k.C, pixels, k.gout, c2.z, mm, k.out, c2.g, nullptr, 0, st));
-    if (bn_sums_needed(h, bd)) RET_IF(vk_bn_bwd_reduce(dt, pixels, k.C, k.gout, cd.z, mm, nullptr, nullptr, k.out, bd.bsums, st));
+    if (bn_sums_needed(h, bd)) {
+      vk::StatsReplicaScope rs_(bwd_repl(h, bd));
+      RET_IF(vk_bn_bwd_reduce(dt, pixels, k.C, k.gout, cd.z, mm, nullptr, nullptr, k.out, bd.bsums, st));
+    }
     RET_IF(bn_bwd_phase2(h, bd, k.C, pixels, k.gout, cd.z, mm, k.out, cd.g, nullptr, 0, st));
   }
   const bool into1 = need_from(h, h->bns[c1.bn].rank);
@@ -1361,6 +1385,7 @@
     vk_conv_desc dd = dgrad_desc(h, c1);
     vk_bnr r;
     r.z = pc2.z; r.scale = nullptr; r.shift = nullptr; r.sums = h->bns[pc2.bn].bsums; r.mask = pb.out; r.accumulate = 1;
+    vk::StatsReplicaScope rs_(bwd_repl(h, h->bns[pc2.bn]));
     const int rc = vk_conv_dgrad_fused(&dd, dgrad_weights(h, c1), gin, nullptr, 0, 0, &r, st);
     if (rc == VK_OK) { tail_fused = true; h->tail_prereduced[(size_t)bi - 1] = 1; }
     else if (rc != VK_ERR_UNSUPPORTED) return rc;
diff --git a/vickers-hardness-unet_amd/csrc/vk_common.h b/vickers-hardness-unet_amd/csrc/vk_common.h
--- a/vickers-hardness-unet_amd/csrc/vk_common.h
+++ b/vickers-hardness-unet_amd/csrc/vk_common.h
@@ -272,6 +272,21 @@
 };
 }
 
+namespace vk {
+int stats_replicas();
+struct StatsReplicaScope {
+  int prev;
+  explicit StatsReplicaScope(int r);
+  ~StatsReplicaScope();
+};
+int bn_bwd_coeffs_r(int C, int R, const double* sums, double count, const float* gamma, const float* save_mean, const float* save_invstd,
+                    float* dgamma, float* dbeta, float* coef_abc, hipStream_t st);
+int bn_bwd_apply_fold_r(vk_dtype dtype, size_t pixels, int C, int R, const void* dy, const void* z, int mask_mode, const float* scale,
+                        const float* shift, const void* mask_src, const double* sums, double count, const float* gamma,
+                        const float* save_mean, const float* save_invstd, float* dgamma, float* dbeta, void* dz, void* g_out, int g_acc,
+                        hipStream_t st);
+}
+
 #define VK_CHECK_ARG(cond, ...)                \
   do {                                         \
     if (!(cond)) {                             \
```

Result: no change. 3018 (median of 6 runs) (+0.7%).
